# Ajax0564/VyomAI

Measured on AMD Instinct MI355X. Metric: training tokens/sec (12L d=768 seq=512 GPT-style decoder, CLM), higher is better.
Workload: dtype bf16; 1 GPU; configs[1]: GPT-style Decoder 12L d=768 h=12 RoPE vocab 50265, CLM training B=32/GPU seq=512, AdamW, bf16 kernels + fp32 masters; global_batch=32, seq_len=512, parallelism=dp1, attention=none, weights=deterministic recipe (vyomai_amd.recipe)

## Files before the change

include/vyom_hip.h:

```cpp
#ifndef VYOM_HIP_H
#define VYOM_HIP_H

#include <stdint.h>

#ifdef __cplusplus
extern "C" {
#endif

typedef enum { VY_F32 = 0, VY_BF16 = 1 } vy_dtype;

typedef enum {
  VY_OK = 0,
  VY_ERR_ARG = -1,
  VY_ERR_UNSUPPORTED = -2,
  VY_ERR_LAUNCH = -3
} vy_status;

typedef enum {
  VY_ACT_NONE = 0, VY_ACT_GELU_ERF = 1, VY_ACT_GELU_TANH = 2,
  VY_ACT_SILU = 3, VY_ACT_TANH = 4, VY_ACT_SIGMOID = 5, VY_ACT_RELU6 = 6, VY_ACT_LEAKY_RELU = 7
} vy_act;
#define VY_ACT_SAVE_DERIV 0x100

enum {
// ... 11 lines not shown
int vy_workspace_set(void* stream, void* ws, int64_t bytes);

int vy_linear_fwd(const void* x, int64_t ldx, const void* w, int64_t ldw, const void* bias,
                  const void* residual, int64_t ldr, void* y, int64_t ldy, void* pre_out,
                  int64_t M, int64_t N, int64_t K, int act, int dtype, void* stream);

int vy_qkv_rope_fwd(const void* x, int64_t ldx, const void* w, int64_t ldw, const void* bias,
                    const float* cos_tab, const float* sin_tab, int64_t pos0,
                    void* q, int64_t q_sb, int64_t q_sh, int64_t q_sl,
                    void* k, int64_t k_sb, int64_t k_sh, int64_t k_sl,
                    void* v, int64_t v_sb, int64_t v_sh, int64_t v_sl,
                    int64_t B, int64_t L, int64_t K, int h, int hk, int dh, int dtype,
                    void* stream);

int vy_attn_fwd(const void* q, int64_t q_sb, int64_t q_sh, int64_t q_sl,
                const void* k, int64_t k_sb, int64_t k_sh, int64_t k_sl,
                const void* v, int64_t v_sb, int64_t v_sh, int64_t v_sl,
                void* out, int64_t o_sb, int64_t o_sl, float* lse,
                int mask_kind, int64_t start_pos, const uint8_t* keypad, int64_t kp_sb,
                const float* addmask, int64_t am_sb, int64_t am_sl,
                int64_t B, int h, int hk, int64_t L, int64_t S, int dh, float scale, int dtype,
                void* stream);

int vy_attn_decode(const void* q, int64_t q_sb, int64_t q_sh,
                   const void* k, int64_t k_sb, int64_t k_sh, int64_t k_sl,
                   const void* v, int64_t v_sb, int64_t v_sh, int64_t v_sl,
                   void* out, int64_t o_sb, int64_t B, int h, int hk, int64_t S, int dh,
                   float scale, int dtype, void* stream);

int vy_paged_rope_write(void* qkv, int64_t ld, const int32_t* positions, const int64_t* slot_mapping,
                        const float* cos_tab, const float* sin_tab, int64_t table_rows, void* k_cache,
                        void* v_cache, int64_t max_blocks, int block_size, int64_t T, int h, int hk, int dh,
                        int dtype, void* stream);
int vy_attn_paged_decode(const void* q, int64_t q_ld, const int32_t* q_rows, const void* k_cache,
                         const void* v_cache, int64_t max_blocks, int block_size,
                         const int32_t* block_table, int64_t bt_stride, const int32_t* seqlens,
                         int64_t max_seqlen, void* out, int64_t o_ld, int64_t B, int h, int hk, int dh,
                         float scale, int n_split, void* ws, int64_t ws_bytes, int dtype, void* stream);
int64_t vy_attn_paged_decode_ws_bytes(int64_t B, int h, int hk, int dh, int64_t max_seqlen, int n_split, int dtype);
int vy_paged_gather(const void* k_cache, const void* v_cache, int64_t max_blocks, int block_size,
                    const int32_t* block_table, int64_t n_blocks, int64_t S, void* k_out, void* v_out,
                    int hk, int dh, int dtype, void* stream);

int vy_layernorm_fwd(const void* x, int64_t ldx, const void* gamma, const void* beta, void* y,
                     int64_t ldy, float* mean, float* rstd, int64_t M, int64_t N, float eps,
                     int dtype, void* stream);

int vy_rmsnorm_fwd(const void* x, int64_t ldx, const void* w, void* y, int64_t ldy, int64_t M,
                   int64_t N, float eps, float w_offset, int dtype, void* stream);

int vy_gated_act_fwd(const void* gate_up, int64_t ldg, void* out, int64_t ldo, int64_t M, int64_t I,
                     int act, int dtype, void* stream);

int vy_rmsnorm_bwd(const void* dy, int64_t lddy, const void* x, int64_t ldx, const void* w,
                   const void* add_to, int64_t ldadd, void* dx, int64_t lddx, float* dw, float beta,
                   float* ws, int64_t M, int64_t N, float eps, float w_offset, int dtype, void* stream);

int vy_gated_act_bwd(const void* d_act, int64_t lddo, const void* gate_up, int64_t ldg, void* d_gate_up,
                     int64_t lddg, int64_t M, int64_t I, int act, int dtype, void* stream);

int vy_rope_fwd(void* x, int64_t sb, int64_t sh, int64_t sl, const float* cos_tab,
                const float* sin_tab, int64_t pos0, int64_t B, int heads, int64_t L, int dh,
                int inverse, int dtype, void* stream);


int vy_linear_dgrad(const void* dy, int64_t lddy, const void* wt, int64_t ldwt, const void* pre,
                    int64_t ldpre, int act, const void* add_to, int64_t ldadd, const void* add_to2,
                    int64_t ldadd2, void* dx, int64_t lddx, int64_t M, int64_t N, int64_t K, int dtype,
                    void* stream);

int vy_linear_wgrad(const void* dy, int64_t lddy, const void* x, int64_t ldx, float* dw,
                    int64_t lddw, float* db, float beta, const float* alpha_dev, int64_t M, int64_t N,
                    int64_t K, int dtype, void* stream);

typedef struct vy_wgrad_desc {
  const void* dy; int64_t lddy;
  const void* x; int64_t ldx;
  float* dw; int64_t lddw;
  float* db;
  int64_t M, N, K;
} vy_wgrad_desc;
int vy_linear_wgrad_grouped(const vy_wgrad_desc* descs, int32_t n, int dtype, void* stream);

int64_t vy_layernorm_bwd_ws_rows(int64_t M);
int vy_layernorm_bwd(const void* dy, int64_t lddy, const void* x, int64_t ldx, const void* gamma,
                     const float* mean, const float* rstd, void* dx, int64_t lddx, float* dgamma,
                     float* dbeta, float beta, float* ws, int64_t M, int64_t N, int dtype,
                     void* stream);

int vy_attn_bwd(const void* q, int64_t q_sb, int64_t q_sh, int64_t q_sl,
                const void* k, int64_t k_sb, int64_t k_sh, int64_t k_sl,
                const void* v, int64_t v_sb, int64_t v_sh, int64_t v_sl,
                const void* out, const void* dout, int64_t o_sb, int64_t o_sl, const float* lse,
                float* delta_ws,
                void* dq, int64_t dq_sb, int64_t dq_sh, int64_t dq_sl,
                void* dk, int64_t dk_sb, int64_t dk_sh, int64_t dk_sl,
                void* dv, int64_t dv_sb, int64_t dv_sh, int64_t dv_sl,
                int mask_kind, int64_t start_pos, const uint8_t* keypad, int64_t kp_sb,
                const float* cos_tab, const float* sin_tab, int64_t rope_pos0,
                int64_t B, int h, int hk, int64_t L, int64_t S, int dh, float scale, int dtype,
                void* stream);

int vy_ddp_unique_id(void* id128);
int vy_ddp_init(const void* id128, int rank, int world);
int vy_ddp_world(void);
int vy_ddp_rank(void);
int vy_ddp_all_reduce_async(void* buf, int64_t count, int dtype, void* stream);
int vy_ddp_destroy(void);

int vy_adamw_step(float* p, const float* g, float* m, float* v, void* p_bf16, int64_t n, float lr,
                  float beta1, float beta2, float eps, float weight_decay, int64_t step,
                  float grad_scale, const float* grad_scale_dev, void* stream);
int vy_adamw_step_gated(float* p, const float* g, float* m, float* v, void* p_bf16, int64_t n, float lr,
                        float beta1, float beta2, float eps, float weight_decay, int64_t step,
                        float grad_scale, const float* grad_scale_dev, const float* gate, void* stream);

int vy_sumsq(const float* x, int64_t n, float* out, float* ws, void* stream);

int vy_linear_dropout_fwd(const void* x, int64_t ldx, const void* w, int64_t ldw, const void* bias,
                          const void* residual, int64_t ldr, void* y, int64_t ldy, int64_t M, int64_t N,
                          int64_t K, float p_drop, uint64_t seed, uint64_t offset, int dtype, void* stream);
int vy_dropout(const void* x, int64_t ldx, void* y, int64_t ldy, int64_t M, int64_t N, float p_drop,
               uint64_t seed, uint64_t offset, int dtype, void* stream);

int vy_act_bwd(const void* dy, int64_t lddy, const void* pre, int64_t ldpre, void* dx, int64_t lddx,
               int64_t M, int64_t N, int act, int dtype, void* stream);

int vy_xent_fwd(const void* logits, int64_t ld, const int64_t* labels, int64_t ignore_index, float* lse,
                float* loss_sum, float* count, int64_t M, int64_t V, int32_t* err_flag, int dtype, void* stream);
int vy_xent_bwd(void* logits, int64_t ld, const int64_t* labels, int64_t ignore_index, const float* lse,
                const float* gscale, const float* count, int64_t M, int64_t V, int dtype, void* stream);
int vy_xent_fused(void* logits, int64_t ld, const int64_t* labels, int64_t ignore_index, float* lse,
                  float* loss_sum, const float* count, const float* gscale, int64_t M, int64_t V,
                  int32_t* err_flag, int dtype, void* stream);
int vy_xent_sample_fwd(const void* logits, int64_t ld, const int64_t* labels, int64_t ignore_index, float* lse,
                       float* loss_sum, float* count, int64_t* sampled, float inv_temperature, uint64_t seed,
                       uint64_t offset, int64_t M, int64_t V, int32_t* err_flag, int dtype, void* stream);
int vy_xent_sample_fused(void* logits, int64_t ld, const int64_t* labels, int64_t ignore_index, float* lse,
                         float* loss_sum, const float* count, const float* gscale, int64_t* sampled,
                         float inv_temperature, uint64_t seed, uint64_t offset, int64_t M, int64_t V,
                         int32_t* err_flag, int dtype, void* stream);
int vy_gumbel_noise(float* out, int64_t ld, int64_t M, int64_t V, uint64_t seed, uint64_t offset, void* stream);

int vy_bce_head_fwd(const void* h, int64_t ldh, const void* w, const void* b, float* z, const float* target,
                    const uint8_t* live, float* loss_sum, int64_t M, int64_t d, int dtype, void* stream);
int vy_bce_head_bwd(const void* h, int64_t ldh, const void* w, const float* z, const float* target,
                    const uint8_t* live, const float* gscale, const float* count, void* dh, int64_t lddh, float* dw,
                    float* db, int accumulate, int64_t M, int64_t d, int dtype, void* stream);

int vy_mlm_mask(const int64_t* ids, int64_t n, const int64_t* special_ids, int32_t n_special, float fraction,
                int64_t mask_id, int64_t vocab, int64_t ignore_index, uint64_t seed, uint64_t offset,
                int64_t* masked_ids, int64_t* labels, uint8_t* masked, void* stream);


int vy_logprob_fwd(const void* logits, int64_t ld, const int64_t* labels, const float* weight, float* lse,
                   float* logp, int64_t M, int64_t V, int32_t* err_flag, int dtype, void* stream);
int vy_logprob_bwd(void* logits, int64_t ld, const int64_t* labels, const float* weight, const float* lse,
                   int64_t M, int64_t V, int dtype, void* stream);
int vy_logprob_fused(void* logits, int64_t ld, const int64_t* labels, const float* weight, float* lse,
                     float* logp, int64_t M, int64_t V, int32_t* err_flag, int dtype, void* stream);

int vy_embedding_fwd(const void* table, int64_t ldt, const int64_t* ids, void* out, int64_t ldo,
                     int64_t M, int64_t d, int64_t V, int32_t* err_flag, int dtype, void* stream);
int vy_embedding_bwd(const void* dout, int64_t lddo, const int64_t* ids, float* dw, int64_t lddw,
                     int64_t padding_idx, int64_t M, int64_t d, int64_t V, int dtype, void* stream);

int vy_transpose(const void* in, int64_t ldin, void* out, int64_t ldout, int64_t R, int64_t C,
                 int dtype, void* stream);

typedef struct vy_transpose_desc {
  const void* in; void* out;
// ... 64 lines not shown
```

vyomai_amd/_lib.py:

```python
from __future__ import annotations

import ctypes as C
import os
from typing import Optional

_HERE = os.path.dirname(os.path.abspath(__file__))
LIB_PATH = os.environ.get("VY_LIB_PATH") or os.path.join(_HERE, "lib", "libvyom_hip.so")

VY_F32, VY_BF16 = 0, 1
ACT_NONE, ACT_GELU_ERF, ACT_GELU_TANH = 0, 1, 2
ACT_SILU, ACT_TANH, ACT_SIGMOID, ACT_RELU6, ACT_LEAKY_RELU = 3, 4, 5, 6, 7
ACT_SAVE_DERIV = 0x100
MASK_NONE, MASK_CAUSAL, MASK_KEYPAD, MASK_ADDITIVE = 0, 1, 2, 4

_p, _i64, _i, _f, _u64 = C.c_void_p, C.c_int64, C.c_int, C.c_float, C.c_uint64

PROTOTYPES = {
    "vy_linear_fwd": [_p, _i64, _p, _i64, _p, _p, _i64, _p, _i64, _p, _i64, _i64, _i64, _i, _i, _p],
    "vy_qkv_rope_fwd": [_p, _i64, _p, _i64, _p, _p, _p, _i64,
                        _p, _i64, _i64, _i64, _p, _i64, _i64, _i64, _p, _i64, _i64, _i64,
                        _i64, _i64, _i64, _i, _i, _i, _i, _p],
    "vy_attn_fwd": [_p, _i64, _i64, _i64, _p, _i64, _i64, _i64, _p, _i64, _i64, _i64,
                    _p, _i64, _i64, _p, _i, _i64, _p, _i64, _p, _i64, _i64,
                    _i64, _i, _i, _i64, _i64, _i, _f, _i, _p],
    "vy_attn_decode": [_p, _i64, _i64, _p, _i64, _i64, _i64, _p, _i64, _i64, _i64,
                       _p, _i64, _i64, _i, _i, _i64, _i, _f, _i, _p],
    "vy_paged_rope_write": [_p, _i64, _p, _p, _p, _p, _i64, _p, _p, _i64, _i, _i64, _i, _i, _i, _i, _p],
    "vy_attn_paged_decode": [_p, _i64, _p, _p, _p, _i64, _i, _p, _i64, _p, _i64, _p, _i64, _i64, _i, _i, _i, _f, _i,
                             _p, _i64, _i, _p],
    "vy_paged_gather": [_p, _p, _i64, _i, _p, _i64, _i64, _p, _p, _i, _i, _i, _p],
    "vy_layernorm_fwd": [_p, _i64, _p, _p, _p, _i64, _p, _p, _i64, _i64, _f, _i, _p],
    "vy_rmsnorm_fwd": [_p, _i64, _p, _p, _i64, _i64, _i64, _f, _f, _i, _p],
    "vy_gated_act_fwd": [_p, _i64, _p, _i64, _i64, _i64, _i, _i, _p],
    "vy_rmsnorm_bwd": [_p, _i64, _p, _i64, _p, _p, _i64, _p, _i64, _p, _f, _p, _i64, _i64, _f, _f, _i, _p],
    "vy_gated_act_bwd": [_p, _i64, _p, _i64, _p, _i64, _i64, _i64, _i, _i, _p],
    "vy_rope_fwd": [_p, _i64, _i64, _i64, _p, _p, _i64, _i64, _i, _i64, _i, _i, _i, _p],
    "vy_linear_dgrad": [_p, _i64, _p, _i64, _p, _i64, _i, _p, _i64, _p, _i64, _p, _i64, _i64, _i64, _i64, _i, _p],
    "vy_linear_wgrad": [_p, _i64, _p, _i64, _p, _i64, _p, _f, _p, _i64, _i64, _i64, _i, _p],
    "vy_linear_wgrad_grouped": [_p, _i, _i, _p],
    "vy_layernorm_bwd": [_p, _i64, _p, _i64, _p, _p, _p, _p, _i64, _p, _p, _f, _p, _i64, _i64, _i, _p],
    "vy_attn_bwd": [_p, _i64, _i64, _i64, _p, _i64, _i64, _i64, _p, _i64, _i64, _i64,
                    _p, _p, _i64, _i64, _p, _p,
                    _p, _i64, _i64, _i64, _p, _i64, _i64, _i64, _p, _i64, _i64, _i64,
                    _i, _i64, _p, _i64, _p, _p, _i64, _i64, _i, _i, _i64, _i64, _i, _f, _i, _p],
    "vy_adamw_step": [_p, _p, _p, _p, _p, _i64, _f, _f, _f, _f, _f, _i64, _f, _p, _p],
    "vy_adamw_step_gated": [_p, _p, _p, _p, _p, _i64, _f, _f, _f, _f, _f, _i64, _f, _p, _p, _p],
    "vy_sumsq": [_p, _i64, _p, _p, _p],
    "vy_linear_dropout_fwd": [_p, _i64, _p, _i64, _p, _p, _i64, _p, _i64, _i64, _i64, _i64, _f, _u64, _u64, _i, _p],
    "vy_dropout": [_p, _i64, _p, _i64, _i64, _i64, _f, _u64, _u64, _i, _p],
    "vy_act_bwd": [_p, _i64, _p, _i64, _p, _i64, _i64, _i64, _i, _i, _p],
    "vy_xent_fwd": [_p, _i64, _p, _i64, _p, _p, _p, _i64, _i64, _p, _i, _p],
    "vy_xent_bwd": [_p, _i64, _p, _i64, _p, _p, _p, _i64, _i64, _i, _p],
    "vy_xent_fused": [_p, _i64, _p, _i64, _p, _p, _p, _p, _i64, _i64, _p, _i, _p],
    "vy_xent_sample_fwd": [_p, _i64, _p, _i64, _p, _p, _p, _p, _f, _u64, _u64, _i64, _i64, _p, _i, _p],
    "vy_xent_sample_fused": [_p, _i64, _p, _i64, _p, _p, _p, _p, _p, _f, _u64, _u64, _i64, _i64, _p, _i, _p],
    "vy_gumbel_noise": [_p, _i64, _i64, _i64, _u64, _u64, _p],
    "vy_bce_head_fwd": [_p, _i64, _p, _p, _p, _p, _p, _p, _i64, _i64, _i, _p],
    "vy_bce_head_bwd": [_p, _i64, _p, _p, _p, _p, _p, _p, _p, _i64, _p, _p, _i, _i64, _i64, _i, _p],
    "vy_mlm_mask": [_p, _i64, _p, _i, _f, _i64, _i64, _i64, _u64, _u64, _p, _p, _p, _p],
    "vy_logprob_fwd": [_p, _i64, _p, _p, _p, _p, _i64, _i64, _p, _i, _p],
    "vy_logprob_bwd": [_p, _i64, _p, _p, _p, _i64, _i64, _i, _p],
    "vy_logprob_fused": [_p, _i64, _p, _p, _p, _p, _i64, _i64, _p, _i, _p],
    "vy_transpose_batched": [_p, _i, _i, _i, _p],
    "vy_embedding_fwd": [_p, _i64, _p, _p, _i64, _i64, _i64, _i64, _p, _i, _p],
    "vy_embedding_bwd": [_p, _i64, _p, _p, _i64, _i64, _i64, _i64, _i64, _i, _p],
    "vy_transpose": [_p, _i64, _p, _i64, _i64, _i64, _i, _p],
    "vy_greedy_step": [_p, _i64, _i64, _i64, _i, _p, _i64, _i64, _p, _i64, _p, _i, _p, _p, _p],
    "vy_sampling_probs": [_p, _i64, _i64, _i64, _i, _f, _i, _f, _p, _i64, _p],
    "vy_decoder_step": [_p, _p, _i64, _p, _p, _p, _i64, _p],
    "vy_gemma_decoder_step": [_p, _p, _i64, _p, _i64, _p],
    "vy_cast": [_p, _p, _i64, _i, _i, _p],
    "vy_ddp_unique_id": [_p],
    "vy_ddp_init": [_p, _i, _i],
    "vy_ddp_all_reduce_async": [_p, _i64, _i, _p],
    "vy_ddp_destroy": [],
    "vy_set_concurrent_chains": [_i],
    "vy_workspace_set": [_p, _p, _i64],
}
OTHER_SYMBOLS = ["vy_last_error", "vy_abi_version", "vy_layernorm_bwd_ws_rows", "vy_decode_ws_bytes",
                 "vy_gemma_ws_bytes", "vy_ddp_world", "vy_ddp_rank", "vy_attn_paged_decode_ws_bytes"]
ALL_SYMBOLS = list(PROTOTYPES) + OTHER_SYMBOLS


class VyWgradDesc(C.Structure):
    _fields_ = [("dy", _p), ("lddy", _i64), ("x", _p), ("ldx", _i64), ("dw", _p), ("lddw", _i64), ("db", _p),
                ("M", _i64), ("N", _i64), ("K", _i64)]


class VyomHipError(RuntimeError):
    pass


_lib: Optional[C.CDLL] = None


def load() -> C.CDLL:
    global _lib
    if _lib is not None:
        return _lib
    if not os.path.exists(LIB_PATH):
        raise VyomHipError(
            f"{LIB_PATH} is missing: build it with `python -c 'import __graft_entry__ as g; g.build()'` "
            "(hipcc --offload-arch=gfx950).  vyomai_amd has no CPU or PyTorch fallback."
        )
    lib = C.CDLL(LIB_PATH)
    for name, argtypes in PROTOTYPES.items():
        fn = getattr(lib, name)
        fn.argtypes = argtypes
        fn.restype = C.c_int
    lib.vy_last_error.restype = C.c_char_p
    lib.vy_last_error.argtypes = []
    lib.vy_abi_version.restype = C.c_int
    lib.vy_layernorm_bwd_ws_rows.restype = C.c_int64
    lib.vy_layernorm_bwd_ws_rows.argtypes = [_i64]
    lib.vy_decode_ws_bytes.restype = C.c_int64
    lib.vy_decode_ws_bytes.argtypes = [C.c_int32] * 7
    lib.vy_attn_paged_decode_ws_bytes.restype = C.c_int64
    lib.vy_attn_paged_decode_ws_bytes.argtypes = [_i64, _i, _i, _i, _i64, _i, _i]
    _lib = lib
    return lib


def call(name: str, *args) -> None:
    lib = load()
    rc = getattr(lib, name)(*args)
    if rc != 0:
        raise VyomHipError(f"{name} failed ({rc}): {lib.vy_last_error().decode()}")


def dtype_code(torch_dtype) -> int:
    import torch

    if torch_dtype == torch.bfloat16:
        return VY_BF16
    if torch_dtype == torch.float32:
        return VY_F32
    raise VyomHipError(f"vyomai_amd kernels support float32 and bfloat16, got {torch_dtype}")
```

vyomai_amd/autograd_train.py:

```python
from __future__ import annotations

import os

import weakref
from typing import Optional

import torch

from . import _lib, ops
from ._lib import ACT_GELU_ERF, ACT_NONE, VyomHipError
from .layers.attention import _shadow
from .layers.mask import AttnMask
from .layers.positional_embeddings import resolve_freqs

BF16 = torch.bfloat16


WEIGHT_EPOCH = [0]


class _WtRegistry:

    def __init__(self) -> None:
        self.entries = []
# ... 2 lines not shown

    def register(self, owner, key_fn, src_fn, dst):
        e = [weakref.ref(owner), key_fn, src_fn, dst, WEIGHT_EPOCH[0]]
        self.entries.append(e)
        return e

    def refresh(self) -> None:
        ep = WEIGHT_EPOCH[0]
        if self.epoch_done == ep:
            return
        self.epoch_done = ep
        self.entries = [e for e in self.entries if e[0]() is not None]
        live = [e for e in self.entries if e[4] >= ep - 1 and getattr(e[0](), "_vy_wt_key", None) != e[1](e[0]())]
        if not live:
            return
        pairs = [(e[2](e[0]()), e[3]) for e in live]
        for dt in sorted({s_.dtype for s_, _ in pairs}, key=str):
            sub = [(s_, d_) for s_, d_ in pairs if s_.dtype == dt]
            keys = [(s_.data_ptr(), d_.data_ptr()) for s_, d_ in sub]
            batch = self.batches.get(dt)
            if batch is None or batch.keys != keys:
                batch = self.batches[dt] = ops.TransposeBatch(sub)
            batch.run()
        for e in live:
            e[0]()._vy_wt_key = e[1](e[0]())


_WT = _WtRegistry()


def _wt_cached(owner, key_fn, src_fn) -> torch.Tensor:
    view = getattr(owner, "_vy_wt_view", None)
    key = key_fn(owner)
    entry = getattr(owner, "_vy_wt_entry", None)
    if entry is not None:
        entry[4] = WEIGHT_EPOCH[0]
    if view is not None and getattr(owner, "_vy_wt_key", None) == key:
        return view
    src = src_fn(owner)
    if view is not None and view.dtype == src.dtype and view.device == src.device:
        _WT.refresh()
        if owner._vy_wt_key != key:
            ops.transpose(src, view)
            owner._vy_wt_key = key
        return view
    N, K = src.shape
    ld = _row_stride(N)
    view = torch.zeros((K, ld), dtype=src.dtype, device=src.device)[:, :N]
    ops.transpose(src, view)
    owner._vy_wt_view, owner._vy_wt_key = view, key
    owner._vy_wt_entry = _WT.register(owner, key_fn, src_fn, view)
    return view


_ROW_GRANULE = int(os.environ.get("VY_ROW_GRANULE", "64"))


def _row_stride(n: int) -> int:
    g = _ROW_GRANULE
    return (n + g - 1) // g * g


def _wt(param: torch.Tensor, dtype) -> torch.Tensor:
    return _wt_cached(param, lambda p: (p._version, WEIGHT_EPOCH[0], dtype), lambda p: _shadow(p, dtype))


def _direct(p: Optional[torch.Tensor]) -> bool:
    return p is not None and getattr(p, "_vy_direct", False) and p.grad is not None


def _notify(*params) -> None:
    for p in params:
        if p is not None:
            cb = getattr(p, "_vy_ready", None)
            if cb is not None:
                cb(p)


class _WgradGroup:

    TILES = int(os.environ.get("VY_WGRAD_GROUP_TILES", "100"))

    def __init__(self):
        self.items, self.tiles, self.armed = [], 0, False

    def wants(self, dy, w, alpha) -> bool:
        if alpha is not None or not _GROUP_WGRADS:
            return False
        N, K = w.shape
        return dy.numel() // N >= _GROUP_MIN_ROWS and N < 8192 and N * K >= 512 * 512 and K % 8 == 0

    def add(self, dy, x, w, b) -> None:
        self.add_tensors(dy, x, w.grad, None if b is None else b.grad, [p for p in (w, b) if p is not None])

    def add_tensors(self, dy, x, dw, db, members) -> None:
        self.items.append((dy, x, dw, db, members))
        for p in members:
            p._vy_deferred = True
        self.tiles += -(-dw.shape[0] // 256) * -(-dw.shape[1] // 256)
        if not self.armed:
            torch.autograd.Variable._execution_engine.queue_callback(self._end_of_backward)
            self.armed = True
        if self.tiles >= self.TILES or len(self.items) == 8:
            self.flush()

    def flush(self) -> None:
        items, self.items, self.tiles = self.items, [], 0
        if not items:
            return
        ops.linear_wgrad_grouped([(dy, x, dw, db) for dy, x, dw, db, _ in items])
        for *_, members in items:
            for p in members:
                p._vy_deferred = False
            _notify(*members)

    def _end_of_backward(self) -> None:
        self.armed = False
        self.flush()

    def discard(self) -> None:
        for *_, members in self.items:
            for p in members:
                p._vy_deferred = False
        self.items, self.tiles, self.armed = [], 0, False


_GROUP_WGRADS = os.environ.get("VY_WGRAD_GROUP", "1") != "0"
_DEFER_RESIDUALS = os.environ.get("VY_DEFER_RESIDUALS", "1") != "0"
_GROUP_MIN_ROWS = int(os.environ.get("VY_WGRAD_GROUP_ROWS", "2048"))
_GROUP_QKV = os.environ.get("VY_WGRAD_GROUP_QKV", "1") != "0"
_wgrad_group = _WgradGroup()


def _wgrad(dy, x, w: torch.Tensor, b: Optional[torch.Tensor], alpha: Optional[torch.Tensor] = None):
    if _direct(w) and (b is None or _direct(b)):
        if _wgrad_group.wants(dy, w, alpha):
            _wgrad_group.add(dy, x, w, b)
            return None, None
        ops.linear_wgrad(dy, x, w.grad, None if b is None else b.grad, accumulate=True, alpha=alpha)
        _notify(w, b)
        return None, None
    dw = torch.empty(w.shape, dtype=torch.float32, device=w.device)
    db = torch.empty(b.shape, dtype=torch.float32, device=w.device) if b is not None else None
    ops.linear_wgrad(dy, x, dw, db, accumulate=False, alpha=alpha)
    return dw.to(w.dtype), (db.to(b.dtype) if b is not None else None)


def _ln_bwd(dy, x, ln_w, ln_b, mean, rstd):
    dt = x.dtype
    if _direct(ln_w) and _direct(ln_b):
        dx = ops.layernorm_bwd(dy, x, _shadow(ln_w, dt), mean, rstd, ln_w.grad, ln_b.grad, accumulate=True)
        _notify(ln_w, ln_b)
        return dx, None, None
    dg = torch.empty(ln_w.shape, dtype=torch.float32, device=x.device)
    db = torch.empty(ln_b.shape, dtype=torch.float32, device=x.device)
    dx = ops.layernorm_bwd(dy, x, _shadow(ln_w, dt), mean, rstd, dg, db, accumulate=False)
    return dx, dg.to(ln_w.dtype), db.to(ln_b.dtype)


def _defer_list(t: torch.Tensor):
    return getattr(t, "_vy_defer", None) if t is not None else None


def defer_residual_grads(x: torch.Tensor) -> None:
    if torch.is_grad_enabled() and x.requires_grad and _DEFER_RESIDUALS:
        x._vy_defer = []


def _require_bf16(x: torch.Tensor) -> None:
    if x.dtype != BF16 and x.dtype != torch.float32:
        raise VyomHipError("training kernels take bf16 or fp32 activations (fp32 master weights), not %s" % x.dtype)


_EMB_USES = {}
_EMB_WAITING = {}


def reset_embedding_uses() -> None:
    _EMB_USES.clear()
    _EMB_WAITING.clear()


def _embedding_end_of_backward() -> None:
    waiting = list(_EMB_WAITING.values())
    _EMB_WAITING.clear()
    for w in waiting:
        _EMB_USES.pop(id(w), None)
        _notify(w)


class EmbeddingFn(torch.autograd.Function):

    @staticmethod
    def forward(ctx, ids, weight, padding_idx, dtype):
        ctx.save_for_backward(ids)
        ctx.weight, ctx.padding_idx = weight, padding_idx
        if _direct(weight):
            _EMB_USES.setdefault(id(weight), [0, 0])[0] += 1
        return ops.embedding(_shadow(weight, dtype), ids)

    @staticmethod
    def backward(ctx, dout):
        (ids,) = ctx.saved_tensors
        w = ctx.weight
        if _direct(w):
            ops.embedding_bwd_(dout.contiguous(), ids, w.grad, ctx.padding_idx)
            uses = _EMB_USES.get(id(w))
            if uses is not None:
                uses[1] += 1
                if uses[1] < uses[0]:
                    _EMB_WAITING[id(w)] = w
                    torch.autograd.Variable._execution_engine.queue_callback(_embedding_end_of_backward)
                    return None, None, None, None
                del _EMB_USES[id(w)]
                _EMB_WAITING.pop(id(w), None)
            _notify(w)
            return None, None, None, None
        dw = torch.zeros(w.shape, dtype=torch.float32, device=w.device)
        ops.embedding_bwd_(dout.contiguous(), ids, dw, ctx.padding_idx)
        return None, dw.to(w.dtype), None, None


class PatchifyFn(torch.autograd.Function):

    @staticmethod
    def forward(ctx, patches, w, b):
        _require_bf16(patches)
        dt = patches.dtype
        ctx.save_for_backward(patches)
        ctx.params = (w, b)
        return ops.linear(patches, _shadow(w, dt).reshape(w.shape[0], -1), _shadow(b, dt))

    @staticmethod
# ... 756 lines not shown
```

vyomai_amd/csrc/vy_bwd.hip:

```cpp
#include "vy_attn_tile.h"
#include <float.h>
#include <stdlib.h>

namespace {


__device__ __forceinline__ int xcd_remap(int bid, int nwg) {
  const int xcd = bid & 7, q = nwg >> 3, r = nwg & 7;
  return (xcd < r ? xcd * (q + 1) : r * (q + 1) + (xcd - r) * q) + (bid >> 3);
}

__device__ __forceinline__ bf16x8 tr_pair(const char* base, int row_bytes) {
  const s16x4 lo = __builtin_amdgcn_ds_read_tr16_b64_v4i16((VY_LDS s16x4*)(base));
  const s16x4 hi = __builtin_amdgcn_ds_read_tr16_b64_v4i16((VY_LDS s16x4*)(base + 8 * row_bytes));
  union { struct { s16x4 a, b; } s; bf16x8 v; } u;
  u.s.a = lo; u.s.b = hi;
  return u.v;
}

typedef __attribute__((ext_vector_type(2))) __bf16 bf16x2_t;

template <int BT, int MS_, bool MF16>
struct WgradTile {
  static constexpr int MS = MS_;
  static constexpr int NW = BT / 32;
  static constexpr int WKT = BT / 2;
  static constexpr int ROWB = BT * 2;
  static constexpr int TILE = MS * ROWB, STAGE = 2 * TILE;
  static constexpr int PP = TILE / 1024 / NW;
  static_assert(PP * 1024 * NW == TILE, "tile / wave layout mismatch");

  int wave, nst, m_begin, m_end;
  bool ragged;
  int row[PP];
  const bf16* a_ptr[PP]; const bf16* b_ptr[PP];
  int64_t a_step[PP], b_step[PP];
  const bf16* zero;

  __device__ __forceinline__ WgradTile(const bf16* __restrict__ dY, int64_t lddy, const bf16* __restrict__ X, int64_t ldx,
                                       int n0, int k0, int N, int K, int m_begin_, int m_end_, int wave_, int lane) {
    wave = wave_, m_begin = m_begin_, m_end = m_end_;
    nst = (m_end - m_begin + MS - 1) / MS;
    ragged = ((m_end - m_begin) % MS) != 0;
    zero = reinterpret_cast<const bf16*>(vy_zero16);
    sources(dY, lddy, n0, N, lane, a_ptr, a_step);
    sources(X, ldx, k0, K, lane, b_ptr, b_step);
  }
  __device__ __forceinline__ void sources(const bf16* __restrict__ src, int64_t ld, int c0, int C, int lane,
                                          const bf16* (&ptr)[PP], int64_t (&step)[PP]) {
#pragma unroll
    for (int t = 0; t < PP; ++t) {
      const int P = (wave * PP + t) * 1024 + lane * 16;
      const int r = P / ROWB, off = P % ROWB;
      const int col = (off ^ (((r & 3) << 6) | (MF16 ? ((r >> 2) & 1) << 5 : 0))) >> 1;
      const bool ok = c0 + col < C;
      row[t] = r;
      ptr[t] = ok ? src + (int64_t)(m_begin + r) * ld + c0 + col : zero;
      step[t] = ok ? (int64_t)MS * ld : 0;
    }
  }
  __device__ __forceinline__ void issue(const bf16* (&ptr)[PP], const int64_t (&step)[PP], int s, char* dst) {
    const bool tail = ragged && s == nst - 1;
    const int rows = m_end - (m_begin + s * MS);
#pragma unroll
    for (int t = 0; t < PP; ++t) {
      const bf16* p = (tail && row[t] >= rows) ? zero : ptr[t];
      __builtin_amdgcn_global_load_lds((const VY_GLOBAL void*)p, (VY_LDS void*)(dst + (wave * PP + t) * 1024), 16, 0, 0);
      ptr[t] += step[t];
    }
  }
  __device__ __forceinline__ void stage(int s, char* dst) {
    issue(a_ptr, a_step, s, dst);
    issue(b_ptr, b_step, s, dst + TILE);
  }
};

__device__ __forceinline__ float wgrad_db_dot(const bf16x8& a, float s) {
  const bf16x2_t ones2 = {(__bf16)1.0f, (__bf16)1.0f};
  union { bf16x8 v; bf16x2_t h[4]; } u_;
  u_.v = a;
#pragma unroll
  for (int e = 0; e < 4; ++e) s = __builtin_amdgcn_fdot2_f32_bf16(u_.h[e], ones2, s, false);
  return s;
}

// ... 170 lines not shown
    const bool hi = kq >= 2;
#pragma unroll
    for (int i = 0; i < TI; ++i)
#pragma unroll
      for (int jp = 0; jp < JH; ++jp) {
        const int k = kw + 16 * (2 * jp + (hi ? 1 : 0)) + r16;
#pragma unroll
        for (int r = 0; r < 4; ++r) {
          const unsigned x = __builtin_bit_cast(unsigned, acc[i][2 * jp][r] * alpha);
          const unsigned y = __builtin_bit_cast(unsigned, acc[i][2 * jp + 1][r] * alpha);
          auto sw = __builtin_amdgcn_permlane32_swap(x, y, false, false);
          const int nlo = nw + 16 * i + 4 * (kq & 1) + r;
          if (k < K) {
            if (nlo < N) atomicAdd(dW + (int64_t)nlo * lddw + k, __builtin_bit_cast(float, (unsigned)sw[0]));
            if (nlo + 8 < N) atomicAdd(dW + (int64_t)(nlo + 8) * lddw + k, __builtin_bit_cast(float, (unsigned)sw[1]));
          }
        }
      }
  }
};

template <int BN, int BKW, int MS, int NS, bool MF16>
__device__ __forceinline__ void wgrad_tn_bf16_body(
    const bf16* __restrict__ dY, int64_t lddy, const bf16* __restrict__ X, int64_t ldx,
    float* __restrict__ dW, int64_t lddw, float* __restrict__ db, const float* __restrict__ alpha_dev,
    int M, int N, int K, int tiles_k, int tiles_nk, int m_chunk, int diag, int wg) {
  static_assert(BN == BKW && ((BN == 128 && MS == 64 && NS == 2) || (BN == 256 && MS == 32 && NS == 4)),
                "built shapes: 128 x 128 x 64 in 2 stages, 256 x 256 x 32 in 4");
  typedef WgradTile<BN, MS, MF16> Tile;
  typedef std::conditional_t<MF16, WgradMma16<Tile>, WgradMma32<Tile>> Mma;
  constexpr int STAGE = Tile::STAGE, PS = 2 * Tile::PP;
  __shared__ __attribute__((aligned(16))) char smem[NS * STAGE];
  const int tid = threadIdx.x, lane = tid & 63;
  const int wave = __builtin_amdgcn_readfirstlane(tid >> 6);
  const int wn = wave >> 1, wk = wave & 1;
  const int split = wg / tiles_nk, t2 = wg - split * tiles_nk;
  const int tile_n = t2 / tiles_k, tile_k = t2 - tile_n * tiles_k;
  const int n0 = tile_n * BN, k0 = tile_k * BKW;
  const int m_begin = split * m_chunk;
  const int m_end = min(M, m_begin + m_chunk);
  if (m_begin >= m_end) return;

  Tile t(dY, lddy, X, ldx, n0, k0, N, K, m_begin, m_end, wave, lane);
  const bool do_db = db != nullptr && tile_k == 0 && wk == 0;
  Mma mma(smem, lane, wn, wk);
  const int nst = t.nst;
#pragma unroll
  for (int s_ = 0; s_ < NS - 1; ++s_)
    if (s_ < nst) t.stage(s_, smem + s_ * STAGE);
  for (int s = 0; s < nst; ++s) {
    const int younger = min(NS - 2, nst - 1 - s);
    if (younger >= 2) asm volatile("s_waitcnt vmcnt(%0)" ::"n"(2 * PS) : "memory");
    else if (younger == 1) asm volatile("s_waitcnt vmcnt(%0)" ::"n"(PS) : "memory");
    else asm volatile("s_waitcnt vmcnt(0)" ::: "memory");
    __builtin_amdgcn_s_barrier();
    asm volatile("" ::: "memory");
    if (s + NS - 1 < nst) t.stage(s + NS - 1, smem + (s + NS - 1) % NS * STAGE);
    mma.mma_stage(s % NS * STAGE, do_db);
  }
  if (diag == 1) {
    if (mma.acc[0][0][0] == 12345.678f) dW[0] = 1.f;
    return;
  }
  const float alpha = alpha_dev ? *alpha_dev : 1.0f;
  mma.epilogue(dW, lddw, db, do_db, alpha, n0 + wn * 64, k0 + wk * Tile::WKT, N, K);
}

template <int BN, int BKW, int MS, int NS, bool MF16>
__global__ __launch_bounds__(BN * 2, BN == 128 ? 2 : 1) void wgrad_tn_bf16_kernel(
    const bf16* __restrict__ dY, int64_t lddy, const bf16* __restrict__ X, int64_t ldx,
    float* __restrict__ dW, int64_t lddw, float* __restrict__ db, const float* __restrict__ alpha_dev,
    int M, int N, int K, int tiles_k, int tiles_nk, int m_chunk, int diag) {
  wgrad_tn_bf16_body<BN, BKW, MS, NS, MF16>(dY, lddy, X, ldx, dW, lddw, db, alpha_dev, M, N, K, tiles_k, tiles_nk, m_chunk,
                                            diag, xcd_remap(blockIdx.x, gridDim.x));
}

struct WgradItem {
  const bf16* dY; const bf16* X; float* dW; float* db;
  int64_t lddy, ldx, lddw;
  int M, N, K, tiles_k, tiles_nk, m_chunk, item0;
};
struct WgradGroup { WgradItem g[8]; int n; };

template <int BN, int BKW, int MS, int NS, bool MF16>
__global__ __launch_bounds__(BN * 2, 1) void wgrad_tn_bf16_grouped_kernel(WgradGroup grp, int diag) {
  const int id = xcd_remap(blockIdx.x, gridDim.x);
  int d = 0;
#pragma unroll
  for (int i = 1; i < 8; ++i)
    if (i < grp.n && id >= grp.g[i].item0) d = i;
  WgradItem it = grp.g[0];
#pragma unroll
  for (int i = 1; i < 8; ++i)
    if (d == i) it = grp.g[i];
  wgrad_tn_bf16_body<BN, BKW, MS, NS, MF16>(it.dY, it.lddy, it.X, it.ldx, it.dW, it.lddw, it.db, nullptr, it.M, it.N, it.K,
                                            it.tiles_k, it.tiles_nk, it.m_chunk, diag, id - it.item0);
}

__global__ __launch_bounds__(64) void colsum_bf16_kernel(const bf16* __restrict__ dY, int64_t lddy,
                                                         float* __restrict__ db, int M, int N) {
  const int c0 = (blockIdx.x * 64 + threadIdx.x) * 8;
  if (c0 >= N) return;
  const int m0 = blockIdx.y * 256, m1 = min(M, m0 + 256);
  float s[8] = {0, 0, 0, 0, 0, 0, 0, 0};
  for (int m = m0; m < m1; ++m) {
    const bf16x8 v = *reinterpret_cast<const bf16x8*>(dY + (int64_t)m * lddy + c0);
#pragma unroll
    for (int e = 0; e < 8; ++e) s[e] += (float)v[e];
  }
#pragma unroll
  for (int e = 0; e < 8; ++e)
    if (c0 + e < N) atomicAdd(db + c0 + e, s[e]);
}

struct BwdParams {
  const bf16* q; int64_t q_sb, q_sh, q_sl;
  const bf16* k; int64_t k_sb, k_sh, k_sl;
  const bf16* v; int64_t v_sb, v_sh, v_sl;
  const bf16* o; const bf16* dout; int64_t o_sb, o_sl;
  const float* lse; float* delta;
  bf16* dq; int64_t dq_sb, dq_sh, dq_sl;
  bf16* dk; int64_t dk_sb, dk_sh, dk_sl;
  bf16* dv; int64_t dv_sb, dv_sh, dv_sl;
  int mask_kind; int start_pos;
  const uint8_t* keypad; int64_t kp_sb;
  int B, h, hk, L, S;
  float scale;
  const float* cos_tab; const float* sin_tab; int rope_pos0;
};

__global__ __launch_bounds__(256, 3) void attn_bwd_dq_kernel(BwdParams p) {
  constexpr int DH = 64, RB = 128, NS = 3, KPW = 256;
  typedef AttnStage<RB, NS> Stage;
  constexpr int TILE = Stage::TILE;
  __shared__ __attribute__((aligned(16))) char smem[2 * NS * TILE + KPW * 8];
  const AttnLane ln;
  const AttnQBlock blk(p, ln);
  const int wave = ln.wave, fr = ln.fr, fh = ln.fh;
  const int head = blk.head, b = blk.b, q0 = blk.q0, qi = blk.qi, qrow = blk.qrow;
  const bf16 *Q = blk.Q, *Kb = blk.Kb, *Vb = blk.Vb;
  const bf16* dO = p.dout + (int64_t)b * p.o_sb + (int64_t)qrow * p.o_sl + head * DH;
  bf16x8 qf[4], gf[4];
#pragma unroll
  for (int ks = 0; ks < 4; ++ks) {
    qf[ks] = *reinterpret_cast<const bf16x8*>(Q + ks * 16 + fh * 8);
    gf[ks] = *reinterpret_cast<const bf16x8*>(dO + ks * 16 + fh * 8);
  }
  const int64_t stat = ((int64_t)b * p.h + head) * p.L + qrow;
  const float c = p.scale * LOG2E;
  float neg_lse = -p.lse[stat] * LOG2E;
  float neg_delta;
  {
    const bf16* Op = p.o + (int64_t)b * p.o_sb + (int64_t)qrow * p.o_sl + head * DH;
    float acc_ = 0.f;
#pragma unroll
    for (int ks = 0; ks < 4; ++ks) {
      const bf16x8 of = *reinterpret_cast<const bf16x8*>(Op + ks * 16 + fh * 8);
#pragma unroll
      for (int e = 0; e < 8; ++e) acc_ += (float)of[e] * (float)gf[ks][e];
    }
    acc_ += __shfl_xor(acc_, 32, 64);
    neg_delta = -acc_;
    if (fh == 0 && qi < p.L) p.delta[stat] = neg_delta;
  }
  const bool causal = p.mask_kind & VY_MASK_CAUSAL;
  const bool haskp = p.mask_kind & VY_MASK_KEYPAD;
  const uint8_t* kp = haskp ? p.keypad + (int64_t)b * p.kp_sb : nullptr;

  const Stage st_w(ln, SwDual{}, SwRows<RB>{});
// ... 292 lines not shown
    sb[lr][lc] = colsum;
    __syncthreads();
    if (tid < 64 && n0 + tid < N) atomicAdd(db + n0 + tid, alpha * (sb[0][tid] + sb[1][tid] + sb[2][tid] + sb[3][tid]));
  }
}

int wgrad_f32(const char* who, const void* dy, int64_t lddy, const void* x, int64_t ldx, float* dw, int64_t lddw, float* db,
              float beta, const float* alpha_dev, int64_t M, int64_t N, int64_t K, hipStream_t st) {
  if (beta == 0.f) {
    if (hipMemset2DAsync(dw, lddw * sizeof(float), 0, K * sizeof(float), N, st) != hipSuccess)
      VY_FAIL(VY_ERR_LAUNCH, "%s: memset failed", who);
    if (db && hipMemsetAsync(db, 0, N * sizeof(float), st) != hipSuccess) VY_FAIL(VY_ERR_LAUNCH, "%s: memset failed", who);
  }
  const int tiles_k = (int)vy_cdiv(K, 64), tiles = (int)vy_cdiv(N, 64) * tiles_k;
  int64_t splits = vy_cdiv(1024, tiles);
  const int64_t max_splits = vy_cdiv(M, 64);
  if (splits > max_splits) splits = max_splits;
  if (splits < 1) splits = 1;
  const int64_t m_chunk = vy_cdiv(vy_cdiv(M, splits), 16) * 16;
  splits = vy_cdiv(M, m_chunk);
  hipLaunchKernelGGL(wgrad_tn_f32_kernel, dim3((unsigned)(tiles * splits)), dim3(256), 0, st, (const float*)dy, lddy,
                     (const float*)x, ldx, dw, lddw, db, alpha_dev, (int)M, (int)N, (int)K, tiles_k, tiles, (int)m_chunk);
  VY_CHECK_LAUNCH(who);
  return VY_OK;
}

bool wgrad_bf16_operands_ok(const void* dy, int64_t lddy, const void* x, int64_t ldx, int64_t N, int64_t K) {
  return !(K % 8 || lddy % 8 || ldx % 8 || lddy < vy_cdiv(N, 8) * 8 || (uintptr_t)dy % 16 || (uintptr_t)x % 16);
}

struct WgradSplit { int64_t splits, m_chunk; };
WgradSplit wgrad_split(int64_t M, int64_t want) {
  const int64_t max_splits = vy_cdiv(M, 256);
  if (want > max_splits) want = max_splits;
  if (want < 1) want = 1;
  const int64_t m_chunk = vy_cdiv(vy_cdiv(M, want), 64) * 64;
  return {vy_cdiv(M, m_chunk), m_chunk};
}

int wgrad_env(const char* name, int dflt) { const char* e = getenv(name); return e ? atoi(e) : dflt; }

int wgrad_m16() { static const int v = wgrad_env("VY_WGRAD_M16", 1); return v; }
int wgrad_diag() { static const int v = wgrad_env("VY_WGRAD_DIAG", 0); return v; }

}

extern "C" int vy_linear_wgrad(const void* dy, int64_t lddy, const void* x, int64_t ldx, float* dw,
                               int64_t lddw, float* db, float beta, const float* alpha_dev, int64_t M,
                               int64_t N, int64_t K, int dtype, void* stream) {
  const char* who = "vy_linear_wgrad";
  if (dtype != VY_BF16 && dtype != VY_F32) VY_FAIL(VY_ERR_ARG, "%s: bad dtype %d", who, dtype);
  if (!dy || !x || !dw || M <= 0 || N <= 0 || K <= 0) VY_FAIL(VY_ERR_ARG, "%s: bad arguments", who);
  if (dtype == VY_F32) {
    if (beta != 0.f && beta != 1.f) VY_FAIL(VY_ERR_ARG, "%s: beta must be 0 or 1", who);
    return wgrad_f32(who, dy, lddy, x, ldx, dw, lddw, db, beta, alpha_dev, M, N, K, (hipStream_t)stream);
  }
  if (!wgrad_bf16_operands_ok(dy, lddy, x, ldx, N, K))
    VY_FAIL(VY_ERR_ARG, "%s: K and leading dimensions must be multiples of 8 (lddy >= roundup8(N)), operands 16-byte aligned", who);
  if (beta != 0.f && beta != 1.f) VY_FAIL(VY_ERR_ARG, "%s: beta must be 0 or 1", who);
  static const int wv = wgrad_env("VY_WGRAD_VARIANT", -1);
  static const int tgt = wgrad_env("VY_WGRAD_TARGET", 0);
  if (wv != -1 && wv != 0 && wv != 8)
    VY_FAIL(VY_ERR_UNSUPPORTED, "%s: VY_WGRAD_VARIANT=%d was removed (the values left are 0 and 8; unset selects by shape)", who, wv);
  hipStream_t st = (hipStream_t)stream;
  if (beta == 0.f) {
    if (hipMemset2DAsync(dw, lddw * sizeof(float), 0, K * sizeof(float), N, st) != hipSuccess)
      VY_FAIL(VY_ERR_LAUNCH, "%s: memset failed", who);
    if (db && hipMemsetAsync(db, 0, N * sizeof(float), st) != hipSuccess)
      VY_FAIL(VY_ERR_LAUNCH, "%s: memset failed", who);
  }
  const bool big = wv < 0 ? (N >= 8192 && M >= 4096) : wv == 8;
  const int BT = big ? 256 : 128;
  const int tiles_k = (int)vy_cdiv(K, BT), tiles = (int)vy_cdiv(N, BT) * tiles_k;
  const WgradSplit sp = wgrad_split(M, tgt > 0 ? vy_cdiv(tgt, tiles) : big ? 256 / tiles : vy_cdiv(384, tiles));
  const int w16 = wgrad_m16();
  auto kernel = big ? (w16 ? wgrad_tn_bf16_kernel<256, 256, 32, 4, true> : wgrad_tn_bf16_kernel<256, 256, 32, 4, false>)
                    : (w16 >= 2 ? wgrad_tn_bf16_kernel<128, 128, 64, 2, true> : wgrad_tn_bf16_kernel<128, 128, 64, 2, false>);
  hipLaunchKernelGGL(kernel, dim3((unsigned)(tiles * sp.splits)), dim3(BT * 2), 0, st, (const bf16*)dy, lddy, (const bf16*)x,
                     ldx, dw, lddw, db, alpha_dev, (int)M, (int)N, (int)K, tiles_k, tiles, (int)sp.m_chunk, wgrad_diag());
  VY_CHECK_LAUNCH(who);
  return VY_OK;
}

extern "C" int vy_linear_wgrad_grouped(const vy_wgrad_desc* descs, int32_t n, int dtype, void* stream) {
  const char* who = "vy_linear_wgrad_grouped";
  if (dtype != VY_BF16 && dtype != VY_F32) VY_FAIL(VY_ERR_ARG, "%s: bad dtype %d", who, dtype);
  if (!descs || n <= 0 || n > 8) VY_FAIL(VY_ERR_ARG, "%s: 1..8 descriptors", who);
  if (dtype == VY_F32) {
    for (int i = 0; i < n; ++i) {
      const vy_wgrad_desc& d = descs[i];
      if (!d.dy || !d.x || !d.dw || d.M <= 0 || d.N <= 0 || d.K <= 0) VY_FAIL(VY_ERR_ARG, "%s: descriptor %d: bad arguments", who, i);
      if (int rc = wgrad_f32(who, d.dy, d.lddy, d.x, d.ldx, d.dw, d.lddw, d.db, 1.f, nullptr, d.M, d.N, d.K, (hipStream_t)stream)) return rc;
    }
    return VY_OK;
  }
  int64_t tiles_total = 0;
  for (int i = 0; i < n; ++i) {
    const vy_wgrad_desc& d = descs[i];
    if (!d.dy || !d.x || !d.dw || d.M <= 0 || d.N <= 0 || d.K <= 0) VY_FAIL(VY_ERR_ARG, "%s: descriptor %d: bad arguments", who, i);
    if (!wgrad_bf16_operands_ok(d.dy, d.lddy, d.x, d.ldx, d.N, d.K))
      VY_FAIL(VY_ERR_ARG, "%s: descriptor %d: K and leading dimensions must be multiples of 8, operands 16-byte aligned", who, i);
    tiles_total += vy_cdiv(d.N, 256) * vy_cdiv(d.K, 256);
  }
  static const int tgt = wgrad_env("VY_WGRAD_GROUP_TARGET", 256);
  WgradGroup grp;
  grp.n = n;
  int64_t items = 0;
  for (int i = 0; i < n; ++i) {
    const vy_wgrad_desc& d = descs[i];
    const int64_t tiles_k = vy_cdiv(d.K, 256), tiles = vy_cdiv(d.N, 256) * tiles_k;
    const WgradSplit sp = wgrad_split(d.M, tgt / tiles_total);
    WgradItem& it = grp.g[i];
    it.dY = (const bf16*)d.dy; it.X = (const bf16*)d.x; it.dW = d.dw; it.db = d.db;
    it.lddy = d.lddy; it.ldx = d.ldx; it.lddw = d.lddw;
    it.M = (int)d.M; it.N = (int)d.N; it.K = (int)d.K;
    it.tiles_k = (int)tiles_k; it.tiles_nk = (int)tiles; it.m_chunk = (int)sp.m_chunk; it.item0 = (int)items;
    items += tiles * sp.splits;
  }
  for (int i = n; i < 8; ++i) grp.g[i] = grp.g[0];
  auto kernel = wgrad_m16() ? wgrad_tn_bf16_grouped_kernel<256, 256, 32, 4, true> : wgrad_tn_bf16_grouped_kernel<256, 256, 32, 4, false>;
  hipLaunchKernelGGL(kernel, dim3((unsigned)items), dim3(512), 0, (hipStream_t)stream, grp, wgrad_diag());
  VY_CHECK_LAUNCH(who);
  return VY_OK;
}

namespace {

template <int DHP>
struct GenBwd {
  static constexpr int PITCH = (DHP + 8) * 2, KS = DHP / 32, NDB = DHP / 16, CPRW = DHP / 8, CPT = 64 * CPRW / 256;
};

__device__ __forceinline__ float gen_groups_sum(float v) {
  const unsigned u = __builtin_bit_cast(unsigned, v);
  auto s16 = __builtin_amdgcn_permlane16_swap(u, u, false, false);
  v = __builtin_bit_cast(float, (unsigned)s16[0]) + __builtin_bit_cast(float, (unsigned)s16[1]);
  const unsigned w = __builtin_bit_cast(unsigned, v);
  auto s32 = __builtin_amdgcn_permlane32_swap(w, w, false, false);
  return __builtin_bit_cast(float, (unsigned)s32[0]) + __builtin_bit_cast(float, (unsigned)s32[1]);
}

template <int DHP>
__device__ __forceinline__ void gen_stage(char* dst, const bf16* src, int64_t sl, int row0, int nrows, int dh, int tid,
                                          bf16x8 (&reg)[GenBwd<DHP>::CPT]) {
  (void)dst;
  constexpr int CPRW = GenBwd<DHP>::CPRW, CPT = GenBwd<DHP>::CPT;
  const bf16x8 zero8 = {(bf16)0.f, (bf16)0.f, (bf16)0.f, (bf16)0.f, (bf16)0.f, (bf16)0.f, (bf16)0.f, (bf16)0.f};
#pragma unroll
  for (int i = 0; i < CPT; ++i) {
    const int cidx = tid + 256 * i;
    const int row = cidx / CPRW, ch = cidx - row * CPRW;
    const int r = row0 + row;
    const bool ok = ch * 8 < dh && r < nrows;
    reg[i] = ok ? *reinterpret_cast<const bf16x8*>(src + (int64_t)r * sl + ch * 8) : zero8;
  }
}
template <int DHP>
__device__ __forceinline__ void gen_store(char* dst, int tid, const bf16x8 (&reg)[GenBwd<DHP>::CPT]) {
  constexpr int CPRW = GenBwd<DHP>::CPRW, CPT = GenBwd<DHP>::CPT, PITCH = GenBwd<DHP>::PITCH;
#pragma unroll
  for (int i = 0; i < CPT; ++i) {
    const int cidx = tid + 256 * i;
    const int row = cidx / CPRW, ch = cidx - row * CPRW;
    *reinterpret_cast<bf16x8*>(dst + row * PITCH + ch * 16) = reg[i];
  }
}

template <int DHP>
__global__ __launch_bounds__(256) void attn_bwd_gen_dq_kernel(BwdParams p, int dh) {
  typedef GenBwd<DHP> G;
  constexpr int PITCH = G::PITCH, KS = G::KS, NDB = G::NDB, CPT = G::CPT;
  __shared__ __attribute__((aligned(16))) char smem[2 * 64 * PITCH];
  char* kt = smem;
  char* vt = smem + 64 * PITCH;
  const int tid = threadIdx.x, lane = tid & 63;
  const int wave = __builtin_amdgcn_readfirstlane(tid >> 6);
  const int r16 = lane & 15, kq = lane >> 4;
  const int head = (int)blockIdx.x % p.h, b = (int)blockIdx.x / p.h;
  const int kvh = head / (p.h / p.hk);
  const int q0 = ((int)gridDim.y - 1 - (int)blockIdx.y) * 64;
  const int qi = q0 + wave * 16 + r16;
  const int qrow = qi < p.L ? qi : p.L - 1;
  const bf16* Q = p.q + (int64_t)b * p.q_sb + (int64_t)head * p.q_sh + (int64_t)qrow * p.q_sl;
  const bf16* dO = p.dout + (int64_t)b * p.o_sb + (int64_t)qrow * p.o_sl + head * dh;
  const bf16* Op = p.o + (int64_t)b * p.o_sb + (int64_t)qrow * p.o_sl + head * dh;
  const bf16* Kb = p.k + (int64_t)b * p.k_sb + (int64_t)kvh * p.k_sh;
  const bf16* Vb = p.v + (int64_t)b * p.v_sb + (int64_t)kvh * p.v_sh;
  const bool causal = p.mask_kind & VY_MASK_CAUSAL;
  const bool haskp = p.mask_kind & VY_MASK_KEYPAD;
  const uint8_t* kp = haskp ? p.keypad + (int64_t)b * p.kp_sb : nullptr;
  const bf16x8 zero8 = {(bf16)0.f, (bf16)0.f, (bf16)0.f, (bf16)0.f, (bf16)0.f, (bf16)0.f, (bf16)0.f, (bf16)0.f};
  bf16x8 qf[KS], gf[KS];
  float dacc = 0.f;
#pragma unroll
  for (int ks = 0; ks < KS; ++ks) {
    const int d0 = 32 * ks + 8 * kq;
    qf[ks] = d0 < dh ? *reinterpret_cast<const bf16x8*>(Q + d0) : zero8;
    gf[ks] = d0 < dh ? *reinterpret_cast<const bf16x8*>(dO + d0) : zero8;
    const bf16x8 of = d0 < dh ? *reinterpret_cast<const bf16x8*>(Op + d0) : zero8;
#pragma unroll
    for (int e = 0; e < 8; ++e) dacc += (float)of[e] * (float)gf[ks][e];
  }
  const float neg_delta = -gen_groups_sum(dacc);
  const int64_t stat = ((int64_t)b * p.h + head) * p.L + qrow;
  if (kq == 0 && qi < p.L) p.delta[stat] = neg_delta;
  const float c = p.scale * LOG2E;
// ... 447 lines not shown
```

vyomai_amd/csrc/vy_common.h:

```cpp
#pragma once
#include <hip/hip_runtime.h>
#include <type_traits>
#include <stdint.h>
#include <stdio.h>
#include <math.h>
#include "../../include/vyom_hip.h"

typedef __bf16 bf16;
typedef __attribute__((ext_vector_type(8))) __bf16 bf16x8;
typedef __attribute__((ext_vector_type(4))) __bf16 bf16x4;
typedef __attribute__((ext_vector_type(2))) __bf16 bf16x2;
typedef __attribute__((ext_vector_type(4))) short s16x4;
typedef __attribute__((ext_vector_type(16))) float f32x16;
typedef __attribute__((ext_vector_type(4))) float f32x4;
typedef __attribute__((ext_vector_type(2))) float f32x2;
typedef __attribute__((ext_vector_type(4))) unsigned int u32x4;
typedef __attribute__((ext_vector_type(2))) unsigned int u32x2;

#define VY_LDS __attribute__((address_space(3)))
#define VY_GLOBAL __attribute__((address_space(1)))

__device__ __forceinline__ s16x4 vy_lds_tr16(const char* p) {
  s16x4 r;
  asm volatile("ds_read_b64_tr_b16 %0, %1" : "=v"(r) : "v"((unsigned)(uintptr_t)(VY_LDS const char*)p) : "memory");
  return r;
}
template <int OFF>
__device__ __forceinline__ s16x4 vy_lds_tr16_off(unsigned lds_addr) {
  static_assert(OFF >= 0 && OFF < 65536, "ds offset field is 16 bits");
  s16x4 r;
  asm volatile("ds_read_b64_tr_b16 %0, %1 offset:%2" : "=v"(r) : "v"(lds_addr), "n"(OFF) : "memory");
  return r;
}
template <int OFF0, int OFF1>
__device__ __forceinline__ bf16x8 vy_lds_tr16_pair_off(unsigned lds_addr) {
  union { struct { s16x4 a, b; } s; bf16x8 v; } u;
  u.s.a = vy_lds_tr16_off<OFF0>(lds_addr);
  u.s.b = vy_lds_tr16_off<OFF1>(lds_addr);
  return u.v;
}
template <int OFF>
__device__ __forceinline__ bf16x8 vy_lds_read128_off(unsigned lds_addr) {
  static_assert(OFF >= 0 && OFF < 65536, "ds offset field is 16 bits");
  bf16x8 r;
  asm volatile("ds_read_b128 %0, %1 offset:%2" : "=v"(r) : "v"(lds_addr), "n"(OFF) : "memory");
  return r;
}
__device__ __forceinline__ unsigned vy_lds_addr(const char* p) { return (unsigned)(uintptr_t)(VY_LDS const char*)p; }
__device__ __forceinline__ bf16x8 vy_lds_tr16_pair(const char* p0, const char* p1) {
  union { struct { s16x4 a, b; } s; bf16x8 v; } u;
  u.s.a = vy_lds_tr16(p0);
  u.s.b = vy_lds_tr16(p1);
  return u.v;
}
template <int N, typename F>
__device__ __forceinline__ void vy_static_for(F&& f) {
  if constexpr (N > 0) {
    vy_static_for<N - 1>(f);
    f(std::integral_constant<int, N - 1>{});
  }
}
template <typename T>
__device__ __forceinline__ void vy_tie(T& v) { asm volatile("" : "+v"(v)); }
template <int N, typename... T>
__device__ __forceinline__ void vy_lgkm_wait(T&... v) {
  asm volatile("s_waitcnt lgkmcnt(%0)" ::"n"(N) : "memory");
  (vy_tie(v), ...);
}

void vy_set_error(const char* fmt, ...);
#define VY_FAIL(code, ...)      \
  do {                          \
    vy_set_error(__VA_ARGS__);  \
    return (code);              \
  } while (0)
#define VY_CHECK_LAUNCH(name)                                             \
  do {                                                                    \
    hipError_t e_ = hipGetLastError();                                    \
    if (e_ != hipSuccess)                                                 \
      VY_FAIL(VY_ERR_LAUNCH, "%s: %s", name, hipGetErrorString(e_));      \
  } while (0)

static inline int64_t vy_cdiv(int64_t a, int64_t b) { return (a + b - 1) / b; }

static __device__ __attribute__((aligned(16))) uint32_t vy_zero16[4] = {0, 0, 0, 0};

__device__ __forceinline__ float vy_gelu_erf(float x) {
  return 0.5f * x * (1.0f + erff(x * 0.70710678118654752440f));
}
__device__ __forceinline__ float vy_gelu_erf_grad(float x) {
  const float cdf = 0.5f * (1.0f + erff(x * 0.70710678118654752440f));
  const float pdf = 0.39894228040143267794f * __expf(-0.5f * x * x);
  return cdf + x * pdf;
}
__device__ __forceinline__ float vy_gelu_tanh(float x) {
  const float c = 0.79788456080286535588f;
  return 0.5f * x * (1.0f + tanhf(c * (x + 0.044715f * x * x * x)));
}
__device__ __forceinline__ float vy_gelu_tanh_grad(float x) {
  const float c = 0.79788456080286535588f;
  const float u = c * (x + 0.044715f * x * x * x);
  const float t = tanhf(u);
  return 0.5f * (1.0f + t) + 0.5f * x * (1.0f - t * t) * c * (1.0f + 3.0f * 0.044715f * x * x);
}
__device__ __forceinline__ void vy_phi_fast(float x, float& cdf, float& gauss) {
  const float ax = fabsf(x) * 0.70710678118654752440f;
  const float t = __builtin_amdgcn_rcpf(1.0f + 0.3275911f * ax);
  gauss = __expf(-ax * ax);
  float poly = 1.061405429f;
  poly = poly * t - 1.453152027f;
  poly = poly * t + 1.421413741f;
  poly = poly * t - 0.284496736f;
  poly = poly * t + 0.254829592f;
  const float erf_abs = 1.0f - poly * t * gauss;
  cdf = 0.5f * (1.0f + copysignf(erf_abs, x));
}
__device__ __forceinline__ float vy_gelu_erf_fast(float x) {
  float cdf, g;
  vy_phi_fast(x, cdf, g);
  return x * cdf;
}
__device__ __forceinline__ float vy_gelu_erf_grad_fast(float x) {
  float cdf, g;
  vy_phi_fast(x, cdf, g);
  return cdf + x * 0.39894228040143267794f * g;
}

constexpr float VY_LEAKY_SLOPE = 0.01f;
__device__ __forceinline__ float vy_sigmoid(float x) { return 1.0f / (1.0f + expf(-x)); }
__device__ __forceinline__ float vy_sigmoid_fast(float x) { return __builtin_amdgcn_rcpf(1.0f + __expf(-x)); }
__device__ __forceinline__ float vy_tanh_fast(float x) { return 1.0f - 2.0f * __builtin_amdgcn_rcpf(1.0f + __expf(2.0f * x)); }
__device__ __forceinline__ float vy_relu6(float x) { return fminf(fmaxf(x, 0.0f), 6.0f); }
__device__ __forceinline__ float vy_relu6_grad(float x) { return (x > 0.0f && x < 6.0f) ? 1.0f : 0.0f; }
__device__ __forceinline__ float vy_leaky_relu(float x) { return x > 0.0f ? x : VY_LEAKY_SLOPE * x; }
__device__ __forceinline__ float vy_leaky_relu_grad(float x) { return x > 0.0f ? 1.0f : VY_LEAKY_SLOPE; }

constexpr int VY_ACT_RUNTIME = 0x40;

template <int ACT>
__device__ __forceinline__ float vy_act_fwd(float x) {
  static_assert(ACT != VY_ACT_RUNTIME, "resolve the run-time code with vy_act_dispatch first");
  if constexpr (ACT == VY_ACT_GELU_ERF) return vy_gelu_erf(x);
  else if constexpr (ACT == VY_ACT_GELU_TANH) return vy_gelu_tanh(x);
  else if constexpr (ACT == VY_ACT_SILU) return x * vy_sigmoid(x);
  else if constexpr (ACT == VY_ACT_TANH) return tanhf(x);
  else if constexpr (ACT == VY_ACT_SIGMOID) return vy_sigmoid(x);
  else if constexpr (ACT == VY_ACT_RELU6) return vy_relu6(x);
  else if constexpr (ACT == VY_ACT_LEAKY_RELU) return vy_leaky_relu(x);
  else return x;
}
template <int ACT>
__device__ __forceinline__ float vy_act_grad(float x) {
  static_assert(ACT != VY_ACT_RUNTIME, "resolve the run-time code with vy_act_dispatch first");
  if constexpr (ACT == VY_ACT_GELU_ERF) return vy_gelu_erf_grad(x);
  else if constexpr (ACT == VY_ACT_GELU_TANH) return vy_gelu_tanh_grad(x);
  else if constexpr (ACT == VY_ACT_SILU) { const float s = vy_sigmoid(x); return s * (1.0f + x * (1.0f - s)); }
  else if constexpr (ACT == VY_ACT_TANH) { const float t = tanhf(x); return 1.0f - t * t; }
  else if constexpr (ACT == VY_ACT_SIGMOID) { const float s = vy_sigmoid(x); return s * (1.0f - s); }
  else if constexpr (ACT == VY_ACT_RELU6) return vy_relu6_grad(x);
  else if constexpr (ACT == VY_ACT_LEAKY_RELU) return vy_leaky_relu_grad(x);
  else return 1.0f;
}

template <int ACT, typename F>
__device__ __forceinline__ void vy_act_dispatch(int code, F&& f) {
  if constexpr (ACT != VY_ACT_RUNTIME) {
    f(std::integral_constant<int, ACT>{});
// ... 143 lines not shown
```

vyomai_amd/csrc/vy_gemm.hip:

```cpp
#include "vy_common.h"

int vy_rope_qk(void* q, int64_t q_sb, int64_t q_sh, int64_t q_sl, int hq, void* k, int64_t k_sb, int64_t k_sh,
               int64_t k_sl, int hk, const float* cos_tab, const float* sin_tab, int64_t pos0, int64_t B, int64_t L, int dh,
               int dtype, hipStream_t st);

#include <stdlib.h>
#include <mutex>

namespace {


template <typename T> struct Quad;
template <> struct Quad<bf16> {
  static __device__ __forceinline__ void load(const bf16* p, float (&v)[4]) {
    bf16x4 t = *reinterpret_cast<const bf16x4*>(p);
#pragma unroll
    for (int e = 0; e < 4; ++e) v[e] = (float)t[e];
  }
  static __device__ __forceinline__ void store(bf16* p, const float (&v)[4]) {
    bf16x4 t;
#pragma unroll
    for (int e = 0; e < 4; ++e) t[e] = (bf16)v[e];
    *reinterpret_cast<bf16x4*>(p) = t;
  }
};
template <> struct Quad<float> {
  static __device__ __forceinline__ void load(const float* p, float (&v)[4]) {
    f32x4 t = *reinterpret_cast<const f32x4*>(p);
#pragma unroll
    for (int e = 0; e < 4; ++e) v[e] = t[e];
  }
  static __device__ __forceinline__ void store(float* p, const float (&v)[4]) {
    f32x4 t = {v[0], v[1], v[2], v[3]};
    *reinterpret_cast<f32x4*>(p) = t;
  }
};

template <typename T> __device__ __forceinline__ float round_like(float x);
template <> __device__ __forceinline__ float round_like<bf16>(float x) { return vy_round_bf16(x); }
template <> __device__ __forceinline__ float round_like<float>(float x) { return x; }

template <typename T>
struct EpiPlain {
  const T* bias;
  const T* residual; int64_t ldr;
  const T* residual2; int64_t ldr2;
  const T* gradpre;  int64_t ldg;
  T* y;   int64_t ldy;
  T* pre;
  int vec_ok;
  VyDrop drop;
  int wt_store;
  int pre_deriv;
  int act;
};

template <typename T, int ACT, bool GRAD>
__device__ __forceinline__ void epi_plain_quad_act(const EpiPlain<T>& e, float (&v)[4], int64_t m, int n,
                                                   int N) {
  if (n >= N) return;
  const bool full = e.vec_ok && (n + 3 < N);
  if (full) {
    if (e.bias) { float b[4]; Quad<T>::load(e.bias + n, b);
#pragma unroll
      for (int i = 0; i < 4; ++i) v[i] += b[i]; }
    if (e.pre) {
      if (e.pre_deriv) { float dv[4];
#pragma unroll
        for (int i = 0; i < 4; ++i) dv[i] = vy_act_grad<ACT>(round_like<T>(v[i]));
        Quad<T>::store(e.pre + m * e.ldy + n, dv);
      } else Quad<T>::store(e.pre + m * e.ldy + n, v);
    }
    if constexpr (!GRAD) {
#pragma unroll
      for (int i = 0; i < 4; ++i) v[i] = vy_act_fwd<ACT>(v[i]);
      if (e.drop.thr) {
        uint32_t lots[4];
        vy_drop_lots(e.drop, m, n >> 3, lots);
#pragma unroll
        for (int i = 0; i < 4; ++i) v[i] = vy_drop_keep(e.drop, lots, (n & 7) + i) ? round_like<T>(v[i]) * e.drop.scale : 0.f;
      }
    } else {
      if (e.gradpre) { float g[4]; Quad<T>::load(e.gradpre + m * e.ldg + n, g);
#pragma unroll
        for (int i = 0; i < 4; ++i) v[i] *= e.pre_deriv ? g[i] : vy_act_grad<ACT>(g[i]); }
    }
    if (e.residual) { float r[4]; Quad<T>::load(e.residual + m * e.ldr + n, r);
#pragma unroll
      for (int i = 0; i < 4; ++i) v[i] += r[i]; }
    if (e.residual2) { float r[4]; Quad<T>::load(e.residual2 + m * e.ldr2 + n, r);
#pragma unroll
      for (int i = 0; i < 4; ++i) v[i] += r[i]; }
    Quad<T>::store(e.y + m * e.ldy + n, v);
  } else {
#pragma unroll
    for (int i = 0; i < 4; ++i) {
      if (n + i >= N) break;
      float x = v[i];
      if (e.bias) x += VyT<T>::ld(e.bias + n + i);
      if (e.pre) VyT<T>::st(e.pre + m * e.ldy + n + i, e.pre_deriv ? vy_act_grad<ACT>(round_like<T>(x)) : x);
      if constexpr (!GRAD) {
        x = vy_act_fwd<ACT>(x);
        if (e.drop.thr) {
          uint32_t lots[4];
          vy_drop_lots(e.drop, m, (n + i) >> 3, lots);
          x = vy_drop_keep(e.drop, lots, (n + i) & 7) ? round_like<T>(x) * e.drop.scale : 0.f;
        }
      }
      else if (e.gradpre) { const float gg = VyT<T>::ld(e.gradpre + m * e.ldg + n + i); x *= e.pre_deriv ? gg : vy_act_grad<ACT>(gg); }
      if (e.residual) x += VyT<T>::ld(e.residual + m * e.ldr + n + i);
      if (e.residual2) x += VyT<T>::ld(e.residual2 + m * e.ldr2 + n + i);
      VyT<T>::st(e.y + m * e.ldy + n + i, x);
    }
  }
}

template <typename T, int ACT, bool GRAD>
__device__ __forceinline__ void epi_plain_quad(const EpiPlain<T>& e, float (&v)[4], int64_t m, int n,
                                               int N) {
  if constexpr (ACT != VY_ACT_RUNTIME) epi_plain_quad_act<T, ACT, GRAD>(e, v, m, n, N);
  else vy_act_dispatch<ACT>(e.act, [&](auto a) __attribute__((always_inline)) { epi_plain_quad_act<T, decltype(a)::value, GRAD>(e, v, m, n, N); });
}

template <int ACT>
__device__ __forceinline__ float gradpre_factor_fast(float g, int pre_deriv, int code) {
  if constexpr (ACT != VY_ACT_RUNTIME) {
    return pre_deriv ? g : vy_act_grad_fast<ACT>(g);
  } else {
    float r = g;
    if (!pre_deriv) vy_act_dispatch<ACT>(code, [&](auto a) __attribute__((always_inline)) { r = vy_act_grad_fast<decltype(a)::value>(g); });
    return r;
  }
}

template <int ACT>
__device__ __forceinline__ void epi_chunk_act(const EpiPlain<bf16>& ep, float (&v)[8], bool dual, int64_t m, int n, int N) {
  if (dual && ep.pre_deriv) {
// ... 42 lines not shown
  n -= e.nq;
  if (n < e.nkv) return e.k + b * e.k_sb + (n >> 6) * e.k_sh + lkv * e.k_sl + d;
  n -= e.nkv;
  return e.v + b * e.v_sb + (n >> 6) * e.v_sh + lkv * e.v_sl + d;
}

template <typename T>
__device__ __forceinline__ T* qkv_dest(const EpiQkv<T>& e, int64_t b, int64_t l, int n) {
  if (n < e.nq) { const int hd = n / e.dh, d = n - hd * e.dh;
    return e.q + b * e.q_sb + hd * e.q_sh + l * e.q_sl + d; }
  n -= e.nq;
  if (e.pos_dev) l += *e.pos_dev;
  if (n < e.nkv) { const int hd = n / e.dh, d = n - hd * e.dh;
    return e.k + b * e.k_sb + hd * e.k_sh + l * e.k_sl + d; }
  n -= e.nkv;
  const int hd = n / e.dh, d = n - hd * e.dh;
  return e.v + b * e.v_sb + hd * e.v_sh + l * e.v_sl + d;
}


template <typename T>
__device__ __forceinline__ void epi_qkv_pair(const EpiQkv<T>& e, float (&lo)[4], float (&hi)[4],
                                             int64_t m, int n_lo, int N) {
  if (n_lo >= N) return;
  const int64_t b = m / e.L, l = m - b * e.L;
  if (e.bias) {
    float b0[4], b1[4];
    Quad<T>::load(e.bias + n_lo, b0); Quad<T>::load(e.bias + n_lo + 32, b1);
#pragma unroll
    for (int i = 0; i < 4; ++i) { lo[i] += b0[i]; hi[i] += b1[i]; }
  }
  if (e.rope && n_lo < e.nq + e.nkv) {
    const int d = n_lo & 31;
    const int64_t pp = (e.pos_dev ? (int64_t)*e.pos_dev : e.pos0) + l;
    const float* cp = e.cos_tab + pp * 32 + d;
    const float* sp = e.sin_tab + pp * 32 + d;
    const f32x4 c4 = *reinterpret_cast<const f32x4*>(cp);
    const f32x4 s4 = *reinterpret_cast<const f32x4*>(sp);
#pragma unroll
    for (int i = 0; i < 4; ++i) {
      const float c = round_like<T>(c4[i]), s = round_like<T>(s4[i]);
      const float a = round_like<T>(lo[i]), bb = round_like<T>(hi[i]);
      lo[i] = round_like<T>(a * c) - round_like<T>(bb * s);
      hi[i] = round_like<T>(bb * c) + round_like<T>(a * s);
    }
  }
  Quad<T>::store(qkv_dest(e, b, l, n_lo), lo);
  Quad<T>::store(qkv_dest(e, b, l, n_lo + 32), hi);
}

template <typename T>
__device__ __forceinline__ void epi_qkv_quad(const EpiQkv<T>& e, float (&v)[4], int64_t m, int n, int N) {
  if (n >= N) return;
  const int64_t b = m / e.L, l = m - b * e.L;
  if (e.bias) { float b0[4]; Quad<T>::load(e.bias + n, b0);
#pragma unroll
    for (int i = 0; i < 4; ++i) v[i] += b0[i]; }
  Quad<T>::store(qkv_dest(e, b, l, n), v);
}

__device__ unsigned long long vy_gemm_clk[6];
constexpr int VY_KNOB_ROT = 1;
constexpr int VY_KNOB_CLK = 16;
constexpr int VY_KNOB_NO_BAND = 32;
#define VY_CLK_BEGIN(on)                                                         \
  const bool clk_on_ = (on) && blockIdx.x == 0 && threadIdx.x == 0;              \
  unsigned long long clk_c0_ = 0, clk_w0_ = 0, clk_m_ = 0;                       \
  if (clk_on_) { clk_c0_ = clk_m_ = __builtin_readcyclecounter(); clk_w0_ = wall_clock64(); }
#define VY_CLK_MARK(i)                                                           \
  if (clk_on_) {                                                                 \
    const unsigned long long now_ = __builtin_readcyclecounter();                \
    atomicAdd(&vy_gemm_clk[3 + (i)], now_ - clk_m_);                             \
    clk_m_ = now_;                                                               \
  }
#define VY_CLK_END()                                                             \
  if (clk_on_) {                                                                 \
    atomicAdd(&vy_gemm_clk[0], __builtin_readcyclecounter() - clk_c0_);          \
    atomicAdd(&vy_gemm_clk[1], wall_clock64() - clk_w0_);                        \
    atomicAdd(&vy_gemm_clk[2], 1ull);                                            \
  }

int g_chains = 1;
int g_gemm_variant = -2;
inline bool vy_m16_on() {
  static const int v = [] { const char* e = getenv("VY_GEMM_M16"); return e ? atoi(e) : 1; }();
  return v != 0;
}
inline int vy_gemm_variant() {
  if (g_gemm_variant == -2) { const char* e = getenv("VY_GEMM_VARIANT"); g_gemm_variant = e ? atoi(e) : -1; }
  return g_gemm_variant;
}

__device__ __forceinline__ int xcd_remap(int bid, int nwg) {
  const int xcd = bid & 7, q = nwg >> 3, r = nwg & 7;
  return (xcd < r ? xcd * (q + 1) : r * (q + 1) + (xcd - r) * q) + (bid >> 3);
}

__device__ __forceinline__ void tile_of(int bid, int nwg, int tiles_n, int band_on, int& tile_m, int& tile_n) {
  const int tiles_m = nwg / tiles_n;
  if (band_on && tiles_n >= 8 && (tiles_n & 1) == 0 && (tiles_m & 3) == 0 && tiles_m * tiles_n == nwg) {
    const int xcd = bid & 7, i = bid >> 3;
    const int band = xcd & 1, grp = xcd >> 1;
    const int bw = tiles_n >> 1, pg = tiles_m >> 2;
    tile_m = grp * pg + i / bw;
    tile_n = band * bw + i - (i / bw) * bw;
  } else {
    const int wg = xcd_remap(bid, nwg);
    tile_m = wg / tiles_n;
    tile_n = wg - tile_m * tiles_n;
  }
}

constexpr int BK = 64;
constexpr int ROWB = BK * 2;

constexpr int epi_tile_bytes(int BM, int BN, int PASSES) { return (BM / PASSES) * (BN * 2 + 16); }
constexpr bool epi_has_rope_tab(int BM, int BN, int EPI, int PASSES) {
  return EPI == 1 && epi_tile_bytes(BM, BN, PASSES) + (BM / PASSES) * 128 <= 160 * 1024;
}
constexpr int epi_lds_bytes(int BM, int BN, int EPI, int PASSES) {
  return epi_tile_bytes(BM, BN, PASSES) + (epi_has_rope_tab(BM, BN, EPI, PASSES) ? (BM / PASSES) * 128 : 0);
}
constexpr int vy_cmax(int a, int b) { return a > b ? a : b; }

template <int BM, int BN, int WGM, int WGN, bool MF16> struct AccTile {
  typedef f32x16 T32[BN / (32 * WGN)][BM / (32 * WGM)];
  typedef f32x4 T16[BN / (16 * WGN)][BM / (16 * WGM)];
  typedef std::conditional_t<MF16, T16, T32> type;
};

template <int BM, int BN, int WGM, int WGN, int EPI, int ACT, bool GRAD, int PASSES = 1, bool PF_OK = true, bool MF16 = false>
__device__ __forceinline__ void gemm_epilogue(typename AccTile<BM, BN, WGM, WGN, MF16>::type& acc, char* smem,
                                              int m0, int n0, int M, int N, const EpiPlain<bf16>& ep,
                                              const EpiQkv<bf16>& eq) {
  static_assert(!MF16 || PASSES == 1, "the 16 x 16 accumulator layout is staged in one pass");
  constexpr int NW = WGM * WGN, NT = 64 * NW;
  constexpr int TM = BM / (32 * WGM), TN = BN / (32 * WGN);
  constexpr int EROW = BN * 2 + 16;
  constexpr int RP = BM / PASSES;
  static_assert(WGM % PASSES == 0, "a pass must be whole wave rows");
  const int tid = threadIdx.x, lane = tid & 63;
  const int wave = __builtin_amdgcn_readfirstlane(tid >> 6);
  const int wm = wave / WGN, wn = wave % WGN;
  const int fr = lane & 31, fh = lane >> 5;
  constexpr int CPR = BN / 8;
  char* et = smem;

  const int my_pass = (wm * 32 * TM) / RP;
  auto stage_quad = [&](int row, int col, const float (&v)[4]) {
    bf16x4 w;
#pragma unroll
    for (int e = 0; e < 4; ++e) w[e] = (bf16)v[e];
    *reinterpret_cast<bf16x4*>(et + (row - my_pass * RP) * EROW + col * 2) = w;
  };
  const bf16* biasp = EPI == 0 ? ep.bias : eq.bias;
  const bool bias_vec = (reinterpret_cast<uintptr_t>(biasp) & 7) == 0;
  auto bias_quad = [&](int n, float (&bq)[4]) {
    if (biasp && n + 3 < N && bias_vec) {
      const bf16x4 b4 = *reinterpret_cast<const bf16x4*>(biasp + n);
#pragma unroll
      for (int e = 0; e < 4; ++e) bq[e] = (float)b4[e];
    } else {
#pragma unroll
      for (int e = 0; e < 4; ++e) bq[e] = (biasp && n + e < N) ? (float)biasp[n + e] : 0.f;
    }
  };
  auto stage_all = [&](int pass) {
    if constexpr (!MF16) {
      if (PASSES == 1 || pass == my_pass) {
#pragma unroll
        for (int i = 0; i < TN; ++i)
#pragma unroll
          for (int rg = 0; rg < 4; ++rg) {
            float bq[4];
            bias_quad(n0 + wn * 32 * TN + i * 32 + 8 * rg + 4 * fh, bq);
#pragma unroll
            for (int j = 0; j < TM; ++j) {
              float v[4];
#pragma unroll
              for (int e = 0; e < 4; ++e) v[e] = acc[i][j][4 * rg + e] + bq[e];
              stage_quad(wm * 32 * TM + j * 32 + fr, wn * 32 * TN + i * 32 + 8 * rg + 4 * fh, v);
            }
          }
      }
    } else {
      constexpr int TM16 = BM / (16 * WGM), TN16 = BN / (16 * WGN);
      const int r16 = lane & 15, kq = lane >> 4;
#pragma unroll
      for (int i = 0; i < TN16; ++i) {
        float bq[4];
        bias_quad(n0 + wn * 16 * TN16 + 16 * i + 4 * kq, bq);
#pragma unroll
        for (int j = 0; j < TM16; ++j) {
          float v[4];
#pragma unroll
          for (int e = 0; e < 4; ++e) v[e] = acc[i][j][e] + bq[e];
          stage_quad(wm * 16 * TM16 + 16 * j + r16, wn * 16 * TN16 + 16 * i + 4 * kq, v);
        }
      }
    }
  };

  if constexpr (EPI == 0) {
    const bf16* pf_ptr = GRAD ? (ep.gradpre ? ep.gradpre : ep.residual) : ep.residual;
    const int64_t pf_ld = GRAD ? (ep.gradpre ? ep.ldg : ep.ldr) : ep.ldr;
    const bool pf_is_gradpre = GRAD && ep.gradpre != nullptr;
    auto do_chunk = [&](bf16* __restrict__ dst, bool dual, int pass, int c, bool pf, const bf16x8& p8) {
        const int row = c / CPR, cc = c - row * CPR;
        const int64_t m = m0 + pass * RP + row;
        const int n = n0 + cc * 8;
        if (m >= M || n >= N) return;
        const bf16x8 sv = *reinterpret_cast<const bf16x8*>(et + row * EROW + cc * 16);
        float v[8];
#pragma unroll
        for (int e = 0; e < 8; ++e) v[e] = (float)sv[e];
        if (dual && !ep.pre_deriv) {
          if (ep.vec_ok && n + 8 <= N) {
            *reinterpret_cast<bf16x8*>(ep.pre + m * ep.ldy + n) = sv;
          } else {
            for (int e = 0; e < 8 && n + e < N; ++e) ep.pre[m * ep.ldy + n + e] = sv[e];
          }
        }
        if constexpr (!GRAD && ACT != VY_ACT_NONE) {
          if constexpr (ACT != VY_ACT_RUNTIME) epi_chunk_act<ACT>(ep, v, dual, m, n, N);
          else vy_act_dispatch<ACT>(ep.act, [&](auto a) __attribute__((always_inline)) { epi_chunk_act<decltype(a)::value>(ep, v, dual, m, n, N); });
        }
        if constexpr (!GRAD) {
          if (ep.drop.thr) {
            uint32_t lots[4];
            vy_drop_lots(ep.drop, m, n >> 3, lots);
#pragma unroll
            for (int e = 0; e < 8; ++e) v[e] = vy_drop_keep(ep.drop, lots, e) ? v[e] * ep.drop.scale : 0.f;
          }
        }
        if (ep.vec_ok && n + 8 <= N) {
          if constexpr (GRAD) {
            if (ep.gradpre) {
              const bf16x8 g = pf ? p8 : *reinterpret_cast<const bf16x8*>(ep.gradpre + m * ep.ldg + n);
#pragma unroll
              for (int e = 0; e < 8; ++e) v[e] *= gradpre_factor_fast<ACT>((float)g[e], ep.pre_deriv, ep.act);
            }
          }
          if (ep.residual) {
            const bf16x8 r = (pf && !pf_is_gradpre) ? p8 : *reinterpret_cast<const bf16x8*>(ep.residual + m * ep.ldr + n);
#pragma unroll
            for (int e = 0; e < 8; ++e) v[e] += (float)r[e];
          }
          if (ep.residual2) {
            const bf16x8 r = *reinterpret_cast<const bf16x8*>(ep.residual2 + m * ep.ldr2 + n);
#pragma unroll
            for (int e = 0; e < 8; ++e) v[e] += (float)r[e];
          }
          bf16x8 o;
#pragma unroll
          for (int e = 0; e < 8; ++e) o[e] = (bf16)v[e];
          if (ep.wt_store) {
            asm volatile("global_store_dwordx4 %0, %1, off sc1\n\ts_nop 1" ::"v"(dst + m * ep.ldy + n), "v"(o) : "memory");
          } else {
            *reinterpret_cast<bf16x8*>(dst + m * ep.ldy + n) = o;
          }
        } else {
          for (int e = 0; e < 8 && n + e < N; ++e) {
            float x = v[e];
            if constexpr (GRAD) {
              if (ep.gradpre) { const float gg = (float)ep.gradpre[m * ep.ldg + n + e]; x *= gradpre_factor_fast<ACT>(gg, ep.pre_deriv, ep.act); }
            }
            if (ep.residual) x += (float)ep.residual[m * ep.ldr + n + e];
            if (ep.residual2) x += (float)ep.residual2[m * ep.ldr2 + n + e];
            dst[m * ep.ldy + n + e] = (bf16)x;
          }
        }
    };
    constexpr bool PFK = PF_OK && PASSES == 1 && BM * BN == 256 * 192 && (RP * CPR) % NT == 0;
    constexpr int ITERS = PFK ? (RP * CPR) / NT : 1;
    bf16x8 pre8[ITERS];
    const bool pf_on = PFK && pf_ptr != nullptr && ep.vec_ok && m0 + BM <= M && n0 + BN <= N;
    if constexpr (PFK) {
      if (pf_on) {
#pragma unroll
        for (int it = 0; it < ITERS; ++it) {
          const int c = tid + it * NT;
          const int row = c / CPR, cc = c - row * CPR;
          pre8[it] = *reinterpret_cast<const bf16x8*>(pf_ptr + (int64_t)(m0 + row) * pf_ld + n0 + cc * 8);
        }
      }
    }
    auto flush_plain = [&](bf16* __restrict__ dst, bool final_pass, bool dual, int pass) {
      (void)final_pass;
      if constexpr (PFK) {
        if (pf_on) {
#pragma unroll
          for (int it = 0; it < ITERS; ++it) do_chunk(dst, dual, pass, tid + it * NT, true, pre8[it]);
          return;
        }
      }
      const bf16x8 none{};
      for (int c = tid; c < RP * CPR; c += NT) do_chunk(dst, dual, pass, c, false, none);
    };
    const bool dual = !GRAD && ep.pre != nullptr;
#pragma unroll 1
    for (int pass = 0; pass < PASSES; ++pass) {
      stage_all(pass);
      __syncthreads();
      flush_plain(ep.y, true, dual, pass);
      if (pass + 1 < PASSES) __syncthreads();
    }
  } else {
    constexpr bool TAB = epi_has_rope_tab(BM, BN, 1, PASSES);
    char* rt = smem + RP * EROW;
    const bool use_tab = TAB && eq.rope && n0 < eq.nq + eq.nkv;
    const unsigned Lu = (unsigned)eq.L;
    const unsigned b0 = (unsigned)m0 / Lu, l0 = (unsigned)m0 - b0 * Lu;
    const int64_t pdev = eq.pos_dev ? (int64_t)*eq.pos_dev : 0;
    const int64_t pbase = eq.pos_dev ? pdev : eq.pos0;
#pragma unroll 1
    for (int pass = 0; pass < PASSES; ++pass) {
    constexpr int TIT = (RP * 8 + NT - 1) / NT;
    f32x4 tv[TAB ? TIT : 1][2];
    if constexpr (TAB) {
      if (use_tab) {
#pragma unroll
        for (int it = 0; it < TIT; ++it) {
          const int idx = tid + it * NT;
          const int row = idx >> 3, ch = idx & 7;
          if (RP * 8 % NT == 0 || idx < RP * 8) {
            const unsigned t = l0 + (unsigned)(pass * RP + row);
            const unsigned l = t - (t / Lu) * Lu;
            const float* src = (ch < 4 ? eq.cos_tab : eq.sin_tab) + (pbase + l) * 32 + (ch & 3) * 8;
            tv[it][0] = *reinterpret_cast<const f32x4*>(src);
            tv[it][1] = *reinterpret_cast<const f32x4*>(src + 4);
          }
        }
      }
    }
    stage_all(pass);
    if constexpr (TAB) {
      if (use_tab) {
#pragma unroll
        for (int it = 0; it < TIT; ++it) {
          const int idx = tid + it * NT;
          if (RP * 8 % NT == 0 || idx < RP * 8) {
            bf16x8 o;
#pragma unroll
            for (int e = 0; e < 4; ++e) { o[e] = (bf16)tv[it][0][e]; o[4 + e] = (bf16)tv[it][1][e]; }
            *reinterpret_cast<bf16x8*>(rt + idx * 16) = o;
          }
        }
      }
    }
    __syncthreads();
    for (int c = tid; c < RP * CPR; c += NT) {
      const int row = c / CPR, cc = c - row * CPR;
      const int64_t m = m0 + pass * RP + row;
      const int n = n0 + cc * 8;
      if (m >= M || n >= N) continue;
      const unsigned t = l0 + (unsigned)(pass * RP + row);
      const unsigned tq = t / Lu;
      const int64_t b = b0 + tq, l = t - tq * Lu;
      bf16x8 sv = *reinterpret_cast<const bf16x8*>(et + row * EROW + cc * 16);
      if (eq.rope && n < eq.nq + eq.nkv) {
        const bf16x8 pv = *reinterpret_cast<const bf16x8*>(et + row * EROW + (cc ^ 4) * 16);
        const int d = n & 31;
        const bool hi = (n & 32) != 0;
        float cs[8], sn[8];
        if (TAB && use_tab) {
          const bf16x8 c8 = *reinterpret_cast<const bf16x8*>(rt + row * 128 + (d >> 3) * 16);
          const bf16x8 s8 = *reinterpret_cast<const bf16x8*>(rt + row * 128 + 64 + (d >> 3) * 16);
#pragma unroll
          for (int e = 0; e < 8; ++e) { cs[e] = (float)c8[e]; sn[e] = (float)s8[e]; }
        } else {
          const float* cp = eq.cos_tab + (pbase + l) * 32 + d;
          const float* sp = eq.sin_tab + (pbase + l) * 32 + d;
#pragma unroll
          for (int e = 0; e < 8; ++e) { cs[e] = vy_round_bf16(cp[e]); sn[e] = vy_round_bf16(sp[e]); }
        }
#pragma unroll
        for (int e = 0; e < 8; ++e) {
          const float a = (float)sv[e], o = (float)pv[e];
          const float t1 = vy_round_bf16(a * cs[e]);
          const float t2 = vy_round_bf16((hi ? o : -o) * sn[e]);
          sv[e] = (bf16)(t1 + t2);
        }
      }
      if (eq.vec8 && eq.dh == 64) {
        *reinterpret_cast<bf16x8*>(qkv_dest64(eq, b, l, n, l + pdev)) = sv;
// ... 1091 lines not shown
    const int tn = (int)vy_cdiv(N, 128), tm = (int)vy_cdiv(M, 32);
    hipLaunchKernelGGL((gemm_nt_bf16_kernel<32, 128, 1, 4, EPI, ACT, GRAD>), dim3(tm * tn), dim3(256), 0,
                       st, X, ldx, W, ldw, (int)M, (int)N, (int)K, tn, ep, eq, rot);
  } else if (M <= 1024 || (mid_tiles && vy_cdiv(M, 256) * vy_cdiv(N, 192) * g_chains < 160)) {
    const int tn = (int)vy_cdiv(N, 128), tm = (int)vy_cdiv(M, 128);
    static const int mid16 = [] { const char* e = getenv("VY_GEMM_MID16"); return e ? atoi(e) : 1; }();
    static const int rows_on = [] { const char* e = getenv("VY_GEMM_ROWS"); return e ? atoi(e) : 1; }();
    if (mid16 && rows_on && M > 128 && M <= 320) {
      if (M <= 256) launch_mid<256, 128, 4, 2, EPI, ACT, GRAD>(X, ldx, W, ldw, M, N, K, ep, eq, st, 256, rot);
      else launch_mid<320, 128, 4, 2, EPI, ACT, GRAD>(X, ldx, W, ldw, M, N, K, ep, eq, st, 256, rot);
    } else if (mid16)
      launch_mid<128, 128, 2, 2, EPI, ACT, GRAD>(X, ldx, W, ldw, M, N, K, ep, eq, st, 448, rot);
    else
      hipLaunchKernelGGL((gemm_nt_bf16_kernel<128, 128, 2, 2, EPI, ACT, GRAD>), dim3(tm * tn), dim3(256), 0,
                         st, X, ldx, W, ldw, (int)M, (int)N, (int)K, tn, ep, eq, rot);
  } else {
    const int tn = (int)vy_cdiv(N, 192), tm = (int)vy_cdiv(M, 256);
    const int tn2 = (int)vy_cdiv(N, 256);
    switch (large_m_kernel(vy_gemm_variant(), vy_m16_on(), N >= 3072)) {
      case LargeM::K32_256x256:
        hipLaunchKernelGGL((gemm_nt_bf16_kernel<256, 256, 4, 2, EPI, ACT, GRAD>), dim3(tm * tn2), dim3(512), 0,
                           st, X, ldx, W, ldw, (int)M, (int)N, (int)K, tn2, ep, eq, rot);
        break;
      case LargeM::K32_256x192:
        hipLaunchKernelGGL((gemm_nt_bf16_kernel<256, 192, 4, 2, EPI, ACT, GRAD>), dim3(tm * tn), dim3(512), 0,
                           st, X, ldx, W, ldw, (int)M, (int)N, (int)K, tn, ep, eq, rot);
        break;
      case LargeM::M16_256x256:
        hipLaunchKernelGGL((gemm_nt_bf16_m16_kernel<256, 256, 4, 2, EPI, ACT, GRAD>), dim3(tm * tn2), dim3(512), 0,
                           st, X, ldx, W, ldw, (int)M, (int)N, (int)K, tn2, ep, eq, rot);
        break;
      case LargeM::X3M16_256x192:
        hipLaunchKernelGGL((gemm_nt_bf16_x3m16_kernel<192, EPI, ACT, GRAD>), dim3(tm * tn), dim3(512), 0,
                           st, X, ldx, W, ldw, (int)M, (int)N, (int)K, tn, ep, eq, rot);
        break;
    }
  }
  return 0;
}

template <int EPI, int ACT, bool GRAD>
int launch_f32(const float* X, int64_t ldx, const float* W, int64_t ldw, int64_t M, int64_t N,
               int64_t K, const EpiPlain<float>& ep, const EpiQkv<float>& eq, hipStream_t st) {
  const int tn = (int)vy_cdiv(N, 64), tm = (int)vy_cdiv(M, 64);
  hipLaunchKernelGGL((gemm_nt_f32_kernel<EPI, ACT, GRAD>), dim3(tm * tn), dim3(256), 0, st, X, ldx, W,
                     ldw, (int)M, (int)N, (int)K, tn, ep, eq);
  return 0;
}

inline bool aligned_to(const void* p, size_t a) { return (reinterpret_cast<uintptr_t>(p) % a) == 0; }

template <typename T>
int check_operands(const char* who, const void* x, int64_t ldx, const void* w, int64_t ldw, int64_t M,
                   int64_t N, int64_t K) {
  const int vec = 16 / (int)sizeof(T);
  if (!x || !w) VY_FAIL(VY_ERR_ARG, "%s: null operand", who);
  if (M <= 0 || N <= 0 || K <= 0) VY_FAIL(VY_ERR_ARG, "%s: empty problem M=%ld N=%ld K=%ld", who, (long)M, (long)N, (long)K);
  if (M > INT32_MAX || N > INT32_MAX || K > INT32_MAX) VY_FAIL(VY_ERR_ARG, "%s: dimension overflow", who);
  if (K % vec) VY_FAIL(VY_ERR_ARG, "%s: K=%ld must be a multiple of %d", who, (long)K, vec);
  if (ldx % vec || ldw % vec || !aligned_to(x, 16) || !aligned_to(w, 16))
    VY_FAIL(VY_ERR_ARG, "%s: operand rows must be 16-byte aligned (ldx=%ld ldw=%ld)", who, (long)ldx, (long)ldw);
  if (ldx < K || ldw < K) VY_FAIL(VY_ERR_ARG, "%s: leading dimension smaller than K", who);
  return 0;
}

template <typename T>
int linear_impl(const void* x, int64_t ldx, const void* w, int64_t ldw, const void* bias,
                const void* residual, int64_t ldr, const void* gradpre, int64_t ldg, void* y,
                int64_t ldy, void* pre_out, int64_t M, int64_t N, int64_t K, int act, bool grad,
                hipStream_t st, const char* who, const void* residual2 = nullptr, int64_t ldr2 = 0,
                VyDrop drop = VyDrop{}) {
  if (int rc = check_operands<T>(who, x, ldx, w, ldw, M, N, K)) return rc;
  if (!y) VY_FAIL(VY_ERR_ARG, "%s: null output", who);
  if (ldy < N) VY_FAIL(VY_ERR_ARG, "%s: ldy < N", who);
  EpiPlain<T> ep;
  ep.pre_deriv = (act & VY_ACT_SAVE_DERIV) ? 1 : 0;
  act &= ~VY_ACT_SAVE_DERIV;
  ep.act = act;
  ep.bias = (const T*)bias; ep.residual = (const T*)residual; ep.ldr = ldr;
  ep.residual2 = (const T*)residual2; ep.ldr2 = ldr2;
  if (residual2 && !residual) VY_FAIL(VY_ERR_ARG, "%s: add_to2 without add_to", who);
  ep.gradpre = (const T*)gradpre; ep.ldg = ldg; ep.y = (T*)y; ep.ldy = ldy; ep.pre = (T*)pre_out;
  ep.drop = drop;
  static const int wt_env = [] { const char* e = getenv("VY_GEMM_WT_STORE"); return e ? atoi(e) : 1; }();
  ep.wt_store = (wt_env && (int64_t)M * N * (int64_t)sizeof(T) >= (16 << 20)) ? 1 : 0;
  const int ve = 16 / (int)sizeof(T);
  ep.vec_ok = (ldy % ve == 0) && aligned_to(y, 16) && (!bias || aligned_to(bias, 4 * sizeof(T))) &&
              (!residual || (ldr % ve == 0 && aligned_to(residual, 16))) &&
              (!residual2 || (ldr2 % ve == 0 && aligned_to(residual2, 16))) &&
              (!gradpre || (ldg % ve == 0 && aligned_to(gradpre, 16))) &&
              (!pre_out || aligned_to(pre_out, 16));
  EpiQkv<T> eq{};
#define VY_GO(ACT_, GRAD_)                                                                              \
  do {                                                                                                  \
    if constexpr (sizeof(T) == 2)                                                                       \
      launch_bf16<0, ACT_, GRAD_>((const bf16*)x, ldx, (const bf16*)w, ldw, M, N, K,                    \
                                  *reinterpret_cast<EpiPlain<bf16>*>(&ep), *reinterpret_cast<EpiQkv<bf16>*>(&eq), st); \
    else                                                                                                \
      launch_f32<0, ACT_, GRAD_>((const float*)x, ldx, (const float*)w, ldw, M, N, K,                   \
                                 *reinterpret_cast<EpiPlain<float>*>(&ep), *reinterpret_cast<EpiQkv<float>*>(&eq), st); \
  } while (0)
  if (!grad) {
    if (act == VY_ACT_NONE) VY_GO(VY_ACT_NONE, false);
    else if (act == VY_ACT_GELU_ERF) VY_GO(VY_ACT_GELU_ERF, false);
    else if (act == VY_ACT_GELU_TANH) VY_GO(VY_ACT_GELU_TANH, false);
    else if (vy_act_is_runtime(act)) VY_GO(VY_ACT_RUNTIME, false);
    else VY_FAIL(VY_ERR_ARG, "%s: unknown activation %d", who, act);
  } else {
    if (act == VY_ACT_NONE || !gradpre) VY_GO(VY_ACT_NONE, true);
    else if (act == VY_ACT_GELU_ERF) VY_GO(VY_ACT_GELU_ERF, true);
    else if (act == VY_ACT_GELU_TANH) VY_GO(VY_ACT_GELU_TANH, true);
    else if (vy_act_is_runtime(act) && ep.pre_deriv) VY_GO(VY_ACT_NONE, true);
    else if (vy_act_is_runtime(act)) VY_GO(VY_ACT_RUNTIME, true);
    else VY_FAIL(VY_ERR_ARG, "%s: unknown activation %d", who, act);
  }
#undef VY_GO
  VY_CHECK_LAUNCH(who);
  return VY_OK;
}

template <typename T>
int qkv_impl(const void* x, int64_t ldx, const void* w, int64_t ldw, const void* bias,
             const float* cos_tab, const float* sin_tab, int64_t pos0, void* q, int64_t q_sb,
             int64_t q_sh, int64_t q_sl, void* k, int64_t k_sb, int64_t k_sh, int64_t k_sl, void* v,
             int64_t v_sb, int64_t v_sh, int64_t v_sl, int64_t B, int64_t L, int64_t K, int h, int hk,
             int dh, hipStream_t st, const int* pos_dev = nullptr) {
  const char* who = "vy_qkv_rope_fwd";
  const int64_t M = B * L, N = (int64_t)(h + 2 * hk) * dh;
  if (int rc = check_operands<T>(who, x, ldx, w, ldw, M, N, K)) return rc;
  if (!q || !k || !v) VY_FAIL(VY_ERR_ARG, "%s: null output", who);
  if (h <= 0 || hk <= 0 || h % hk) VY_FAIL(VY_ERR_ARG, "%s: h=%d must be a positive multiple of hk=%d", who, h, hk);
  if (dh % 4) VY_FAIL(VY_ERR_ARG, "%s: head_dim %d must be a multiple of 4", who, dh);
  if ((cos_tab == nullptr) != (sin_tab == nullptr)) VY_FAIL(VY_ERR_ARG, "%s: cos/sin must both be given", who);
  const size_t qa = 4 * sizeof(T);
  const int64_t strides[] = {q_sb, q_sh, q_sl, k_sb, k_sh, k_sl, v_sb, v_sh, v_sl};
  for (int64_t s : strides)
    if (s % 4) VY_FAIL(VY_ERR_ARG, "%s: output strides must be multiples of 4 elements", who);
  if (!aligned_to(q, qa) || !aligned_to(k, qa) || !aligned_to(v, qa) || (bias && !aligned_to(bias, qa)))
    VY_FAIL(VY_ERR_ARG, "%s: outputs/bias must be 4-element aligned", who);
  EpiQkv<T> eq;
  eq.bias = (const T*)bias; eq.cos_tab = cos_tab; eq.sin_tab = sin_tab; eq.pos0 = pos0;
  eq.q = (T*)q; eq.q_sb = q_sb; eq.q_sh = q_sh; eq.q_sl = q_sl;
  eq.k = (T*)k; eq.k_sb = k_sb; eq.k_sh = k_sh; eq.k_sl = k_sl;
  eq.v = (T*)v; eq.v_sb = v_sb; eq.v_sh = v_sh; eq.v_sl = v_sl;
  eq.L = (int)L; eq.nq = h * dh; eq.nkv = hk * dh; eq.dh = dh; eq.pos_dev = pos_dev;
  const bool fuse = cos_tab && sizeof(T) == 2 && dh == 64;
  eq.rope = fuse ? 1 : 0;
  {
    bool v8 = dh % 8 == 0 && aligned_to(q, 16) && aligned_to(k, 16) && aligned_to(v, 16);
    for (int64_t st_ : strides) v8 = v8 && (st_ % 8 == 0);
    eq.vec8 = v8 ? 1 : 0;
  }
  EpiPlain<T> ep{};
  if constexpr (sizeof(T) == 2)
    launch_bf16<1, VY_ACT_NONE, false>((const bf16*)x, ldx, (const bf16*)w, ldw, M, N, K,
                                       *reinterpret_cast<EpiPlain<bf16>*>(&ep), *reinterpret_cast<EpiQkv<bf16>*>(&eq), st);
  else
    launch_f32<1, VY_ACT_NONE, false>((const float*)x, ldx, (const float*)w, ldw, M, N, K,
                                      *reinterpret_cast<EpiPlain<float>*>(&ep), *reinterpret_cast<EpiQkv<float>*>(&eq), st);
  VY_CHECK_LAUNCH(who);
  if (cos_tab && !fuse) {
    if (pos_dev) VY_FAIL(VY_ERR_UNSUPPORTED, "%s: device-side position needs the fused RoPE path (bf16, dh == 64)", who);
    const int vdt = sizeof(T) == 2 ? VY_BF16 : VY_F32;
    if (int rc = vy_rope_qk(q, q_sb, q_sh, q_sl, h, k, k_sb, k_sh, k_sl, hk, cos_tab, sin_tab, pos0, B, L, dh, vdt,
                            (hipStream_t)st)) return rc;
  }
  return VY_OK;
}

}

extern "C" int vy_linear_fwd(const void* x, int64_t ldx, const void* w, int64_t ldw, const void* bias,
                             const void* residual, int64_t ldr, void* y, int64_t ldy, void* pre_out,
                             int64_t M, int64_t N, int64_t K, int act, int dtype, void* stream) {
  hipStream_t st = (hipStream_t)stream;
  if (dtype == VY_BF16)
    return linear_impl<bf16>(x, ldx, w, ldw, bias, residual, ldr, nullptr, 0, y, ldy, pre_out, M, N, K, act, false, st, "vy_linear_fwd");
  if (dtype == VY_F32)
    return linear_impl<float>(x, ldx, w, ldw, bias, residual, ldr, nullptr, 0, y, ldy, pre_out, M, N, K, act, false, st, "vy_linear_fwd");
  VY_FAIL(VY_ERR_ARG, "vy_linear_fwd: bad dtype %d", dtype);
}

extern "C" int vy_linear_dropout_fwd(const void* x, int64_t ldx, const void* w, int64_t ldw, const void* bias,
                                     const void* residual, int64_t ldr, void* y, int64_t ldy, int64_t M, int64_t N,
                                     int64_t K, float p_drop, uint64_t seed, uint64_t offset, int dtype, void* stream) {
  hipStream_t st = (hipStream_t)stream;
  if (!(p_drop >= 0.f && p_drop <= 1.f)) VY_FAIL(VY_ERR_ARG, "vy_linear_dropout_fwd: p=%g outside [0, 1]", (double)p_drop);
  const VyDrop d = vy_make_drop(p_drop, seed, offset);
  if (dtype == VY_BF16)
    return linear_impl<bf16>(x, ldx, w, ldw, bias, residual, ldr, nullptr, 0, y, ldy, nullptr, M, N, K, VY_ACT_NONE, false, st, "vy_linear_dropout_fwd", nullptr, 0, d);
  if (dtype == VY_F32)
    return linear_impl<float>(x, ldx, w, ldw, bias, residual, ldr, nullptr, 0, y, ldy, nullptr, M, N, K, VY_ACT_NONE, false, st, "vy_linear_dropout_fwd", nullptr, 0, d);
  VY_FAIL(VY_ERR_ARG, "vy_linear_dropout_fwd: bad dtype %d", dtype);
}

extern "C" int vy_linear_dgrad(const void* dy, int64_t lddy, const void* wt, int64_t ldwt, const void* pre,
                               int64_t ldpre, int act, const void* add_to, int64_t ldadd, const void* add_to2,
                               int64_t ldadd2, void* dx, int64_t lddx, int64_t M, int64_t N, int64_t K, int dtype,
                               void* stream) {
  hipStream_t st = (hipStream_t)stream;
  if (dtype == VY_BF16)
    return linear_impl<bf16>(dy, lddy, wt, ldwt, nullptr, add_to, ldadd, pre, ldpre, dx, lddx, nullptr, M, K, N, act, true, st, "vy_linear_dgrad", add_to2, ldadd2);
  if (dtype == VY_F32)
    return linear_impl<float>(dy, lddy, wt, ldwt, nullptr, add_to, ldadd, pre, ldpre, dx, lddx, nullptr, M, K, N, act, true, st, "vy_linear_dgrad", add_to2, ldadd2);
  VY_FAIL(VY_ERR_ARG, "vy_linear_dgrad: bad dtype %d", dtype);
}

extern "C" int vy_qkv_rope_fwd(const void* x, int64_t ldx, const void* w, int64_t ldw, const void* bias,
                               const float* cos_tab, const float* sin_tab, int64_t pos0, void* q,
                               int64_t q_sb, int64_t q_sh, int64_t q_sl, void* k, int64_t k_sb,
                               int64_t k_sh, int64_t k_sl, void* v, int64_t v_sb, int64_t v_sh,
                               int64_t v_sl, int64_t B, int64_t L, int64_t K, int h, int hk, int dh,
                               int dtype, void* stream) {
  hipStream_t st = (hipStream_t)stream;
  if (dtype == VY_BF16)
    return qkv_impl<bf16>(x, ldx, w, ldw, bias, cos_tab, sin_tab, pos0, q, q_sb, q_sh, q_sl, k, k_sb, k_sh, k_sl, v, v_sb, v_sh, v_sl, B, L, K, h, hk, dh, st);
  if (dtype == VY_F32)
    return qkv_impl<float>(x, ldx, w, ldw, bias, cos_tab, sin_tab, pos0, q, q_sb, q_sh, q_sl, k, k_sb, k_sh, k_sl, v, v_sb, v_sh, v_sl, B, L, K, h, hk, dh, st);
  VY_FAIL(VY_ERR_ARG, "vy_qkv_rope_fwd: bad dtype %d", dtype);
}

int64_t vy_splitk_ws_floats(int64_t N) { return 8 * 32 * N; }

extern "C" int vy_debug_set_gemm_variant(int v) { g_gemm_variant = v; return 0; }
extern "C" int vy_workspace_set(void* stream, void* ws, int64_t bytes) {
  if (bytes < 0 || (ws && ((uintptr_t)ws & 255))) VY_FAIL(VY_ERR_ARG, "vy_workspace_set: bad workspace (256-byte aligned, bytes >= 0)");
  std::lock_guard<std::mutex> lk(g_ws_mu);
  hipStream_t st = (hipStream_t)stream;
  for (int i = 0; i < g_ws_n; ++i)
    if (g_ws[i].st == st) {
      if (ws && bytes) { g_ws[i].p = ws; g_ws[i].bytes = bytes; }
      else { g_ws[i] = g_ws[g_ws_n - 1]; --g_ws_n; }
      return VY_OK;
    }
  if (!ws || !bytes) return VY_OK;
  if (g_ws_n == 16) {
    for (int i = 1; i < 16; ++i) g_ws[i - 1] = g_ws[i];
    --g_ws_n;
  }
  g_ws[g_ws_n++] = WsEntry{st, ws, bytes};
  return VY_OK;
}
extern "C" int vy_set_concurrent_chains(int n) {
  if (n < 1 || n > 8) VY_FAIL(VY_ERR_ARG, "vy_set_concurrent_chains: n = %d (1..8)", n);
  g_chains = n;
  return VY_OK;
}

extern "C" int vy_debug_gemm_clock(unsigned long long* out3) {
  unsigned long long z[6] = {0, 0, 0, 0, 0, 0};
  if (hipMemcpyFromSymbol(out3, HIP_SYMBOL(vy_gemm_clk), sizeof(z)) != hipSuccess) return 1;
  return hipMemcpyToSymbol(HIP_SYMBOL(vy_gemm_clk), z, sizeof(z)) != hipSuccess;
}
int vy_linear_res_ln_skinny(const void* x, int64_t ldx, const void* w, int64_t ldw, const void* bias,
                            const void* residual, int64_t ldr, const void* gamma, const void* beta, float eps,
                            void* y, int64_t ldy, float* part, int64_t M, int64_t N, int64_t K, void* stream) {
  const char* who = "vy_linear_res_ln_skinny";
  if (!x || !w || !gamma || !beta || !y || !part) VY_FAIL(VY_ERR_ARG, "%s: null operand", who);
  if (M < 1 || M > 32 || N % 32 || K % 16 || N > 8192) VY_FAIL(VY_ERR_UNSUPPORTED, "%s: needs M <= 32, N %% 32 == 0 (<= 8192), K %% 16 == 0", who);
  if (ldx % 8 || ldw % 8 || ldy % 8 || (residual && ldr % 8)) VY_FAIL(VY_ERR_ARG, "%s: strides must be multiples of 8", who);
  hipStream_t st = (hipStream_t)stream;
  const int nsteps = (int)(K / 16), nwg = (int)(N / 32);
  int ksplit = (256 + nwg - 1) / nwg;
  if (ksplit > 8) ksplit = 8;
  if (ksplit > nsteps / 8) ksplit = nsteps / 8;
  if (ksplit < 1) ksplit = 1;
  int spw = (nsteps + ksplit - 1) / ksplit;
  spw = (spw + 3) / 4 * 4;
  ksplit = (nsteps + spw - 1) / spw;
  hipLaunchKernelGGL(gemm_skinny_splitk_kernel, dim3((unsigned)nwg, (unsigned)ksplit), dim3(256), 0, st, (const bf16*)x,
                     ldx, (const bf16*)w, ldw, (int)M, (int)N, (int)K, spw, part);
  VY_CHECK_LAUNCH(who);
  static const int row_fin = [] { const char* e = getenv("VY_DECODE_ROW_FINISH"); return e ? atoi(e) : 1; }();
  if (row_fin && N % 4 == 0) {
    const int qpt = (int)vy_cdiv(N / 4, 256);
#define ROW_GO(Q)                                                                                               \
    hipLaunchKernelGGL((splitk_finish_ln_row_kernel<Q>), dim3((unsigned)M), dim3(256), 0, st, part, ksplit, (int)M, (int)N, \
                       (const bf16*)bias, (const bf16*)residual, ldr, (const bf16*)gamma, (const bf16*)beta, (bf16*)y, ldy, eps)
    if (qpt <= 1) ROW_GO(1);
    else if (qpt <= 2) ROW_GO(2);
    else if (qpt <= 4) ROW_GO(4);
    else ROW_GO(8);
#undef ROW_GO
    VY_CHECK_LAUNCH(who);
    return VY_OK;
  }
  const int nch = (int)(N / 8);
  const dim3 grid((unsigned)((M + 3) / 4)), block(256);
#define FIN_GO(CH)                                                                                               \
  hipLaunchKernelGGL((splitk_finish_ln_kernel<CH>), grid, block, 0, st, part, ksplit, (int)M, (int)N, (const bf16*)bias, \
                     (const bf16*)residual, ldr, (const bf16*)gamma, (const bf16*)beta, (bf16*)y, ldy, eps)
  if (nch <= 64) FIN_GO(1);
  else if (nch <= 128) FIN_GO(2);
  else if (nch <= 256) FIN_GO(4);
  else if (nch <= 512) FIN_GO(8);
  else FIN_GO(16);
#undef FIN_GO
  VY_CHECK_LAUNCH(who);
  return VY_OK;
}

#define VY_NORM_PRESCALED ((const void*)(intptr_t)-1)
static bool gemv_ok(const void* x, int64_t ldx, const void* w, int64_t ldw, int64_t M, int64_t K) {
  return M >= 1 && M <= 4 && K % 8 == 0 && ldx % 8 == 0 && ldw % 8 == 0 && ((uintptr_t)x % 16 == 0) && ((uintptr_t)w % 16 == 0);
}
int vy_gemv_norm(const void* x, int64_t ldx, const void* w, int64_t ldw, const void* bias, const void* norm_w, float eps,
                 const void* residual, int64_t ldr, void* y, int64_t ldy, int64_t M, int64_t N, int64_t K, void* stream) {
// ... 80 lines not shown
```

vyomai_amd/csrc/vy_misc.hip:

```cpp
#include "vy_common.h"
#include <stdarg.h>
#include <string.h>

static thread_local char g_err[512] = "";
void vy_set_error(const char* fmt, ...) {
  va_list ap;
  va_start(ap, fmt);
  vsnprintf(g_err, sizeof(g_err), fmt, ap);
  va_end(ap);
}
extern "C" const char* vy_last_error(void) { return g_err; }
extern "C" int vy_abi_version(void) { return 5; }

namespace {

template <typename T, int CH>
__global__ __launch_bounds__(256) void layernorm_fwd_kernel(const T* __restrict__ x, int64_t ldx,
                                                            const T* __restrict__ gamma,
                                                            const T* __restrict__ beta, T* __restrict__ y,
                                                            int64_t ldy, float* __restrict__ mean_out,
                                                            float* __restrict__ rstd_out, int64_t M, int N,
                                                            float eps) {
  constexpr int VEC = Chunk<T>::VEC;
  const int lane = threadIdx.x & 63;
// ... 704 lines not shown
    if (c < nch) {
      bf16x8 o;
#pragma unroll
      for (int e = 0; e < 8; ++e) {
        const int col = c * 8 + e;
        float g = 0.f;
        if (col < V) g = p.grad(s, __expf((float)v[i][e] - l), col == label ? 1.f : 0.f);
        o[e] = (bf16)g;
      }
      *reinterpret_cast<bf16x8*>(row + (int64_t)c * 8) = o;
    }
  }
}

int row_check(const char* fn, bool ptrs, const void* logits, int64_t ld, int64_t M, int64_t V, int dtype, const char* pair) {
  if (!ptrs || M <= 0 || V <= 0) VY_FAIL(VY_ERR_ARG, "%s: bad arguments", fn);
  if (pair) {
    if (dtype != VY_BF16) VY_FAIL(VY_ERR_UNSUPPORTED, "%s: bf16 only (use %s)", fn, pair);
    if (V > 65536) VY_FAIL(VY_ERR_UNSUPPORTED, "%s: V=%ld exceeds the 65536 columns a workgroup keeps in registers (use %s)", fn, (long)V, pair);
    if (ld % 8 || ld < vy_cdiv(V, 8) * 8 || (uintptr_t)logits % 16) VY_FAIL(VY_ERR_ARG, "%s: rows must be 16-byte aligned and cover the padded width", fn);
    return VY_OK;
  }
  const int vec = dtype == VY_BF16 ? 8 : 4;
  if (ld % vec || ld < vy_cdiv(V, vec) * vec) VY_FAIL(VY_ERR_ARG, "%s: row stride must be a multiple of %d and cover the padded row", fn, vec);
  if (dtype != VY_BF16 && dtype != VY_F32) VY_FAIL(VY_ERR_ARG, "%s: bad dtype %d", fn, dtype);
  return VY_OK;
}

template <typename P>
int row_lse(const char* fn, bool ptrs, const void* logits, int64_t ld, const int64_t* labels, const P& p, float* lse,
            int64_t M, int64_t V, int32_t* err, int dtype, void* stream) {
  if (const int rc = row_check(fn, ptrs && logits && labels && lse, logits, ld, M, V, dtype, nullptr)) return rc;
  const dim3 grid((unsigned)M), block(256);
  if (dtype == VY_BF16) hipLaunchKernelGGL((row_lse_kernel<bf16, P>), grid, block, 0, (hipStream_t)stream, (const bf16*)logits, ld, labels, p, lse, (int)V, err);
  else hipLaunchKernelGGL((row_lse_kernel<float, P>), grid, block, 0, (hipStream_t)stream, (const float*)logits, ld, labels, p, lse, (int)V, err);
  VY_CHECK_LAUNCH(fn);
  return VY_OK;
}

template <typename P>
int row_grad(const char* fn, bool ptrs, void* logits, int64_t ld, const int64_t* labels, const P& p, const float* lse,
             int64_t M, int64_t V, int dtype, void* stream) {
  if (const int rc = row_check(fn, ptrs && logits && labels && lse, logits, ld, M, V, dtype, nullptr)) return rc;
  const dim3 grid((unsigned)M), block(256);
  if (dtype == VY_BF16) hipLaunchKernelGGL((row_grad_kernel<bf16, P>), grid, block, 0, (hipStream_t)stream, (bf16*)logits, ld, labels, p, lse, (int)V);
  else hipLaunchKernelGGL((row_grad_kernel<float, P>), grid, block, 0, (hipStream_t)stream, (float*)logits, ld, labels, p, lse, (int)V);
  VY_CHECK_LAUNCH(fn);
  return VY_OK;
}

template <typename P>
int row_fused(const char* fn, bool ptrs, void* logits, int64_t ld, const int64_t* labels, const P& p, float* lse,
              int64_t M, int64_t V, int32_t* err, int dtype, void* stream) {
  if (const int rc = row_check(fn, ptrs && logits && labels && lse, logits, ld, M, V, dtype, P::kPair)) return rc;
  hipLaunchKernelGGL((row_fused_kernel<P>), dim3((unsigned)M), dim3(1024), 0, (hipStream_t)stream, (bf16*)logits, ld, labels, p, lse, (int)V, err);
  VY_CHECK_LAUNCH(fn);
  return VY_OK;
}

template <typename T>
int ln_fwd_dispatch(const void* x, int64_t ldx, const void* gamma, const void* beta, void* y, int64_t ldy,
                    float* mean, float* rstd, int64_t M, int64_t N, float eps, hipStream_t st) {
  constexpr int VEC = Chunk<T>::VEC;
  if (N % VEC || ldx % VEC || ldy % VEC) VY_FAIL(VY_ERR_ARG, "vy_layernorm_fwd: N/ld must be multiples of %d", VEC);
  const int nch = (int)(N / VEC);
  const dim3 grid((unsigned)vy_cdiv(M, 4)), block(256);
#define LN_GO(CH)                                                                                       \
  hipLaunchKernelGGL((layernorm_fwd_kernel<T, CH>), grid, block, 0, st, (const T*)x, ldx, (const T*)gamma, \
                     (const T*)beta, (T*)y, ldy, mean, rstd, M, (int)N, eps)
  if (nch <= 64) LN_GO(1);
  else if (nch <= 128) LN_GO(2);
  else if (nch <= 256) LN_GO(4);
  else if (nch <= 512) LN_GO(8);
  else if (nch <= 1024) LN_GO(16);
  else VY_FAIL(VY_ERR_UNSUPPORTED, "vy_layernorm_fwd: N=%ld too wide", (long)N);
#undef LN_GO
  VY_CHECK_LAUNCH("vy_layernorm_fwd");
  return VY_OK;
}

template <typename T>
int ln_bwd_dispatch(const void* dy, int64_t lddy, const void* x, int64_t ldx, const void* gamma,
                    const float* mean, const float* rstd, void* dx, int64_t lddx, float* dgamma,
                    float* dbeta, float beta, float* ws, int64_t M, int64_t N, hipStream_t st) {
  constexpr int VEC = Chunk<T>::VEC;
  if (N % VEC || ldx % VEC || lddy % VEC || lddx % VEC) VY_FAIL(VY_ERR_ARG, "vy_layernorm_bwd: N/ld must be multiples of %d", VEC);
  const int nch = (int)(N / VEC);
  const int WB = (int)vy_layernorm_bwd_ws_rows(M);
  const int W = WB * 4;
  const dim3 grid((unsigned)WB), block(256);
#define LN_GO(CH)                                                                                        \
  hipLaunchKernelGGL((layernorm_bwd_kernel<T, CH>), grid, block, 0, st, (const T*)dy, lddy, (const T*)x, ldx, \
                     (const T*)gamma, mean, rstd, (T*)dx, lddx, ws, M, (int)N, W)
  if (nch <= 64) LN_GO(1);
  else if (nch <= 128) LN_GO(2);
  else if (nch <= 256) LN_GO(4);
  else VY_FAIL(VY_ERR_UNSUPPORTED, "vy_layernorm_bwd: N=%ld too wide", (long)N);
#undef LN_GO
  VY_CHECK_LAUNCH("vy_layernorm_bwd");
  if (beta != 0.f && beta != 1.f) VY_FAIL(VY_ERR_ARG, "vy_layernorm_bwd: beta must be 0 or 1");
  const int acc = beta == 1.f;
  const int slices = WB >= 64 ? 16 : 1;
  const int rps = (int)vy_cdiv(WB, slices);
  hipLaunchKernelGGL(colsum_partials_kernel, dim3((unsigned)vy_cdiv(N, 64), (unsigned)slices), dim3(256), 0, st, ws, WB,
                     (int)N, dgamma, dbeta, rps, acc);
  VY_CHECK_LAUNCH("vy_layernorm_bwd(colsum)");
  if (slices > 1) {
    hipLaunchKernelGGL(colsum_finish_kernel, dim3((unsigned)vy_cdiv(N, 256)), dim3(256), 0, st, ws, WB, (int)N, dgamma,
                       dbeta, rps, acc);
    VY_CHECK_LAUNCH("vy_layernorm_bwd(colsum finish)");
  }
  return VY_OK;
}

}

extern "C" int vy_layernorm_fwd(const void* x, int64_t ldx, const void* gamma, const void* beta, void* y,
                                int64_t ldy, float* mean, float* rstd, int64_t M, int64_t N, float eps,
                                int dtype, void* stream) {
  if (!x || !gamma || !beta || !y || M <= 0 || N <= 0) VY_FAIL(VY_ERR_ARG, "vy_layernorm_fwd: bad arguments");
  hipStream_t st = (hipStream_t)stream;
  if (dtype == VY_BF16) return ln_fwd_dispatch<bf16>(x, ldx, gamma, beta, y, ldy, mean, rstd, M, N, eps, st);
  if (dtype == VY_F32) return ln_fwd_dispatch<float>(x, ldx, gamma, beta, y, ldy, mean, rstd, M, N, eps, st);
  VY_FAIL(VY_ERR_ARG, "vy_layernorm_fwd: bad dtype %d", dtype);
}

extern "C" int vy_rmsnorm_fwd(const void* x, int64_t ldx, const void* w, void* y, int64_t ldy, int64_t M, int64_t N,
                              float eps, float w_offset, int dtype, void* stream) {
  if (!x || !w || !y || M <= 0 || N <= 0) VY_FAIL(VY_ERR_ARG, "vy_rmsnorm_fwd: bad arguments");
  hipStream_t st = (hipStream_t)stream;
  const int vec = dtype == VY_BF16 ? 8 : 4;
  if (N % vec || ldx % vec || ldy % vec) VY_FAIL(VY_ERR_ARG, "vy_rmsnorm_fwd: N/ld must be multiples of %d", vec);
  const int nch = (int)(N / vec);
  const dim3 grid((unsigned)vy_cdiv(M, 4)), block(256);
#define RMS_GO(T, CH) hipLaunchKernelGGL((rmsnorm_fwd_kernel<T, CH>), grid, block, 0, st, (const T*)x, ldx, (const T*)w, (T*)y, ldy, M, (int)N, eps, w_offset)
#define RMS_DISPATCH(T)                                  \
  if (nch <= 64) RMS_GO(T, 1);                           \
  else if (nch <= 128) RMS_GO(T, 2);                     \
  else if (nch <= 256) RMS_GO(T, 4);                     \
  else if (nch <= 512) RMS_GO(T, 8);                     \
  else if (nch <= 1024) RMS_GO(T, 16);                   \
  else VY_FAIL(VY_ERR_UNSUPPORTED, "vy_rmsnorm_fwd: N=%ld too wide", (long)N)
  if (dtype == VY_BF16) { RMS_DISPATCH(bf16); }
  else if (dtype == VY_F32) { RMS_DISPATCH(float); }
  else VY_FAIL(VY_ERR_ARG, "vy_rmsnorm_fwd: bad dtype %d", dtype);
#undef RMS_DISPATCH
#undef RMS_GO
  VY_CHECK_LAUNCH("vy_rmsnorm_fwd");
  return VY_OK;
}

extern "C" int vy_gated_act_fwd(const void* gate_up, int64_t ldg, void* out, int64_t ldo, int64_t M, int64_t I, int act,
                                int dtype, void* stream) {
  if (!gate_up || !out || M <= 0 || I <= 0) VY_FAIL(VY_ERR_ARG, "vy_gated_act_fwd: bad arguments");
  if (dtype != VY_BF16 && dtype != VY_F32) VY_FAIL(VY_ERR_ARG, "vy_gated_act_fwd: bad dtype %d", dtype);
  if (act != VY_ACT_GELU_ERF && act != VY_ACT_GELU_TANH && !vy_act_is_runtime(act))
    VY_FAIL(VY_ERR_ARG, "vy_gated_act_fwd: unsupported act %d", act);
  hipStream_t st = (hipStream_t)stream;
  const int vec = dtype == VY_BF16 ? 8 : 4;
  if (I % vec || ldg % vec || ldo % vec) VY_FAIL(VY_ERR_ARG, "vy_gated_act_fwd: I/ld must be multiples of %d", vec);
  const int64_t want = vy_cdiv(M * (I / vec), 256);
  const dim3 grid((unsigned)(want < 8192 ? want : 8192)), block(256);
#define GA_GO(T, A) hipLaunchKernelGGL((gated_act_kernel<T, A>), grid, block, 0, st, (const T*)gate_up, ldg, (T*)out, ldo, M, (int)I, act)
  if (dtype == VY_BF16 && act == VY_ACT_GELU_TANH) GA_GO(bf16, VY_ACT_GELU_TANH);
  else if (dtype == VY_BF16 && act == VY_ACT_GELU_ERF) GA_GO(bf16, VY_ACT_GELU_ERF);
  else if (dtype == VY_F32 && act == VY_ACT_GELU_TANH) GA_GO(float, VY_ACT_GELU_TANH);
  else if (dtype == VY_F32 && act == VY_ACT_GELU_ERF) GA_GO(float, VY_ACT_GELU_ERF);
  else if (dtype == VY_BF16) GA_GO(bf16, VY_ACT_RUNTIME);
  else GA_GO(float, VY_ACT_RUNTIME);
#undef GA_GO
  VY_CHECK_LAUNCH("vy_gated_act_fwd");
  return VY_OK;
}

extern "C" int64_t vy_layernorm_bwd_ws_rows(int64_t M) {
  static const int64_t cap = [] { const char* e = getenv("VY_LNBWD_WB"); return e ? (int64_t)atoi(e) : (int64_t)512; }();
  const int64_t b = (M + 3) / 4;
  return b < 1 ? 1 : (b > cap ? cap : b);
}

extern "C" int vy_layernorm_bwd(const void* dy, int64_t lddy, const void* x, int64_t ldx, const void* gamma,
                                const float* mean, const float* rstd, void* dx, int64_t lddx, float* dgamma,
                                float* dbeta, float beta, float* ws, int64_t M, int64_t N, int dtype,
                                void* stream) {
  if (!dy || !x || !gamma || !mean || !rstd || !dx || !ws || M <= 0 || N <= 0)
    VY_FAIL(VY_ERR_ARG, "vy_layernorm_bwd: bad arguments");
  hipStream_t st = (hipStream_t)stream;
  if (dtype == VY_BF16) return ln_bwd_dispatch<bf16>(dy, lddy, x, ldx, gamma, mean, rstd, dx, lddx, dgamma, dbeta, beta, ws, M, N, st);
  if (dtype == VY_F32) return ln_bwd_dispatch<float>(dy, lddy, x, ldx, gamma, mean, rstd, dx, lddx, dgamma, dbeta, beta, ws, M, N, st);
  VY_FAIL(VY_ERR_ARG, "vy_layernorm_bwd: bad dtype %d", dtype);
}

int vy_rope_qk(void* q, int64_t q_sb, int64_t q_sh, int64_t q_sl, int hq, void* k, int64_t k_sb, int64_t k_sh,
               int64_t k_sl, int hk, const float* cos_tab, const float* sin_tab, int64_t pos0, int64_t B, int64_t L, int dh,
               int dtype, hipStream_t st) {
  if (!q || !k || !cos_tab || !sin_tab || (dh & 1)) VY_FAIL(VY_ERR_ARG, "vy_rope_qk: bad arguments");
  const int64_t total = B * (hq > hk ? hq : hk) * L * (dh / 2);
  const dim3 grid((unsigned)vy_cdiv(total, 256), 2), block(256);
  if (dtype == VY_BF16)
    hipLaunchKernelGGL(rope2_kernel<bf16>, grid, block, 0, st, (bf16*)q, q_sb, q_sh, q_sl, hq, (bf16*)k, k_sb, k_sh, k_sl, hk,
                       cos_tab, sin_tab, pos0, B, L, dh);
  else if (dtype == VY_F32)
    hipLaunchKernelGGL(rope2_kernel<float>, grid, block, 0, st, (float*)q, q_sb, q_sh, q_sl, hq, (float*)k, k_sb, k_sh, k_sl,
                       hk, cos_tab, sin_tab, pos0, B, L, dh);
  else VY_FAIL(VY_ERR_ARG, "vy_rope_qk: bad dtype %d", dtype);
  VY_CHECK_LAUNCH("vy_rope_qk");
  return VY_OK;
}

extern "C" int vy_rope_fwd(void* x, int64_t sb, int64_t sh, int64_t sl, const float* cos_tab,
                           const float* sin_tab, int64_t pos0, int64_t B, int heads, int64_t L, int dh,
                           int inverse, int dtype, void* stream) {
  if (!x || !cos_tab || !sin_tab || dh % 2 || B <= 0 || heads <= 0 || L <= 0)
    VY_FAIL(VY_ERR_ARG, "vy_rope_fwd: bad arguments");
  hipStream_t st = (hipStream_t)stream;
  const int64_t total = B * heads * L * (dh / 2);
  const dim3 grid((unsigned)vy_cdiv(total, 256)), block(256);
  if (dtype == VY_BF16)
    hipLaunchKernelGGL(rope_kernel<bf16>, grid, block, 0, st, (bf16*)x, sb, sh, sl, cos_tab, sin_tab, pos0, B, heads, L, dh, inverse);
  else if (dtype == VY_F32)
    hipLaunchKernelGGL(rope_kernel<float>, grid, block, 0, st, (float*)x, sb, sh, sl, cos_tab, sin_tab, pos0, B, heads, L, dh, inverse);
  else VY_FAIL(VY_ERR_ARG, "vy_rope_fwd: bad dtype %d", dtype);
  VY_CHECK_LAUNCH("vy_rope_fwd");
  return VY_OK;
}

extern "C" int vy_act_bwd(const void* dy, int64_t lddy, const void* pre, int64_t ldpre, void* dx, int64_t lddx,
                          int64_t M, int64_t N, int act, int dtype, void* stream) {
  if (!dy || !pre || !dx || M <= 0 || N <= 0) VY_FAIL(VY_ERR_ARG, "vy_act_bwd: bad arguments");
  hipStream_t st = (hipStream_t)stream;
  const int vec = dtype == VY_BF16 ? 8 : 4;
  if (N % vec || lddy % vec || ldpre % vec || lddx % vec) VY_FAIL(VY_ERR_ARG, "vy_act_bwd: N/ld must be multiples of %d", vec);
  const int64_t want = vy_cdiv(M * (N / vec), 256);
  const dim3 grid((unsigned)(want < 8192 ? want : 8192)), block(256);
#define AB_GO(T, A) hipLaunchKernelGGL((act_bwd_kernel<T, A>), grid, block, 0, st, (const T*)dy, lddy, (const T*)pre, ldpre, (T*)dx, lddx, M, (int)N)
  if (dtype == VY_BF16 && act == VY_ACT_GELU_ERF) AB_GO(bf16, VY_ACT_GELU_ERF);
  else if (dtype == VY_BF16 && act == VY_ACT_GELU_TANH) AB_GO(bf16, VY_ACT_GELU_TANH);
  else if (dtype == VY_F32 && act == VY_ACT_GELU_ERF) AB_GO(float, VY_ACT_GELU_ERF);
  else if (dtype == VY_F32 && act == VY_ACT_GELU_TANH) AB_GO(float, VY_ACT_GELU_TANH);
#define AB_CODE(A)                                          \
  else if (dtype == VY_BF16 && act == A) AB_GO(bf16, A);    \
  else if (dtype == VY_F32 && act == A) AB_GO(float, A);
  AB_CODE(VY_ACT_SILU) AB_CODE(VY_ACT_TANH) AB_CODE(VY_ACT_SIGMOID) AB_CODE(VY_ACT_RELU6) AB_CODE(VY_ACT_LEAKY_RELU)
#undef AB_CODE
  else VY_FAIL(VY_ERR_ARG, "vy_act_bwd: unsupported act %d / dtype %d", act, dtype);
#undef AB_GO
  VY_CHECK_LAUNCH("vy_act_bwd");
  return VY_OK;
}

extern "C" int vy_xent_fwd(const void* logits, int64_t ld, const int64_t* labels, int64_t ignore_index, float* lse,
                           float* loss_sum, float* count, int64_t M, int64_t V, int32_t* err_flag, int dtype,
                           void* stream) {
  return row_lse("vy_xent_fwd", loss_sum && count, logits, ld, labels,
                 XentRow<true>{ignore_index, nullptr, nullptr, loss_sum, count}, lse, M, V, err_flag, dtype, stream);
}

extern "C" int vy_xent_bwd(void* logits, int64_t ld, const int64_t* labels, int64_t ignore_index, const float* lse,
                           const float* gscale, const float* count, int64_t M, int64_t V, int dtype, void* stream) {
  return row_grad("vy_xent_bwd", gscale && count, logits, ld, labels,
                  XentRow<false>{ignore_index, gscale, count, nullptr, nullptr}, lse, M, V, dtype, stream);
}

extern "C" int vy_xent_fused(void* logits, int64_t ld, const int64_t* labels, int64_t ignore_index, float* lse,
                             float* loss_sum, const float* count, const float* gscale, int64_t M, int64_t V,
                             int32_t* err_flag, int dtype, void* stream) {
  return row_fused("vy_xent_fused", loss_sum && count && gscale, logits, ld, labels,
                   XentRow<false>{ignore_index, gscale, count, loss_sum, nullptr}, lse, M, V, err_flag, dtype, stream);
}

extern "C" int vy_xent_sample_fwd(const void* logits, int64_t ld, const int64_t* labels, int64_t ignore_index,
                                  float* lse, float* loss_sum, float* count, int64_t* sampled, float inv_temperature,
                                  uint64_t seed, uint64_t offset, int64_t M, int64_t V, int32_t* err_flag, int dtype,
                                  void* stream) {
  XentSampleRow<true> p{{ignore_index, nullptr, nullptr, loss_sum, count}, sampled, inv_temperature, vy_make_noise(seed, offset)};
// ... 306 lines not shown
```

vyomai_amd/ops.py:

```python
from __future__ import annotations

import math
from typing import Optional, Tuple

import torch

from . import _lib
from ._lib import call, dtype_code

Tensor = torch.Tensor




class _Lanes:
    active = False
    side: Optional[torch.cuda.Stream] = None
    fork_ev: Optional[torch.cuda.Event] = None
    join_ev: Optional[torch.cuda.Event] = None
    B = L = B0 = 0
    dirty = False
    keep: list = []
    streams = {}


class lanes:

    def __init__(self, B: int, L: int, enabled: bool = True):
        self.on = bool(enabled) and B >= 2 and not _Lanes.active and torch.cuda.is_available()
        self.B, self.L = B, L

    def __enter__(self):
        if self.on:
            dev = torch.cuda.current_device()
            st = _Lanes.streams.get(dev)
            if st is None:
                st = _Lanes.streams[dev] = (torch.cuda.Stream(), torch.cuda.Event(), torch.cuda.Event())
            _Lanes.side, _Lanes.fork_ev, _Lanes.join_ev = st
            _Lanes.B, _Lanes.L, _Lanes.B0 = self.B, self.L, self.B // 2
            _Lanes.active, _Lanes.dirty, _Lanes.keep = True, False, []
            call("vy_set_concurrent_chains", 2)
        return self

    def __exit__(self, *exc):
        if self.on:
            _lanes_join()
            _Lanes.active = False
            call("vy_set_concurrent_chains", 1)
            if _Lanes.keep:
                _Lanes.keep = []
        return False


def _lanes_join() -> None:
    if _Lanes.active and _Lanes.dirty:
        _Lanes.join_ev.record(_Lanes.side)
        torch.cuda.current_stream().wait_event(_Lanes.join_ev)
        _Lanes.dirty = False


def _lane_plan(rows: Optional[int] = None, batches: Optional[int] = None, keep=()):
    main = torch.cuda.current_stream()
    if _Lanes.active:
        if rows is not None and rows == _Lanes.B * _Lanes.L:
            cut, n = _Lanes.B0 * _Lanes.L, rows
        elif batches is not None and batches == _Lanes.B:
            cut, n = _Lanes.B0, batches
        else:
            cut = None
        if cut is not None:
            _Lanes.fork_ev.record(main)
            _Lanes.side.wait_event(_Lanes.fork_ev)
            _Lanes.dirty = True
            if keep:
                _Lanes.keep.extend(t for t in keep if t is not None)
            return [(0, cut, main.cuda_stream), (cut, n - cut, _Lanes.side.cuda_stream)]
        _lanes_join()
    n = rows if rows is not None else batches
    return [(0, n, main.cuda_stream)]


def _stream() -> int:
    _lanes_join()
    return torch.cuda.current_stream().cuda_stream


# ... 144 lines not shown
    B, h, _, dh = q.shape
    hk = k.shape[1]
    out = torch.empty((B, 1, h * dh), dtype=q.dtype, device=q.device)
    if scale is None:
        scale = 1.0 / math.sqrt(dh)
    call("vy_attn_decode", q.data_ptr(), q.stride(0), q.stride(1),
         k.data_ptr(), k.stride(0), k.stride(1), k.stride(2),
         v.data_ptr(), v.stride(0), v.stride(1), v.stride(2),
         out.data_ptr(), out.stride(0), B, h, hk, S, dh, float(scale), dtype_code(q.dtype), _stream())
    return out


def layernorm(x: Tensor, gamma: Tensor, beta: Tensor, eps: float,
              save_stats: bool = False) -> Tuple[Tensor, Optional[Tensor], Optional[Tensor]]:
    _need_gpu(x, gamma, beta)
    x2 = _rows(x)
    M, N = x2.shape
    y = torch.empty((M, N), dtype=x.dtype, device=x.device)
    mean = rstd = None
    if save_stats:
        mean = torch.empty(M, dtype=torch.float32, device=x.device)
        rstd = torch.empty(M, dtype=torch.float32, device=x.device)
    whole = _Lanes.active and x2.data_ptr() != x.data_ptr()
    for m0, m, st in ([(0, M, _stream())] if whole else _lane_plan(rows=M, keep=(x2, y, mean, rstd, gamma, beta))):
        call("vy_layernorm_fwd", _at(x2, m0), x2.stride(0), gamma.data_ptr(), beta.data_ptr(),
             _at(y, m0), y.stride(0), _at(mean, m0), _at(rstd, m0), m, N, float(eps), dtype_code(x.dtype), st)
    return y.view(x.shape), mean, rstd


def rope_(x: Tensor, cos: Tensor, sin: Tensor, pos0: int = 0, inverse: bool = False) -> Tensor:
    _need_gpu(x, cos, sin)
    B, heads, L, dh = x.shape
    assert x.stride(3) == 1
    call("vy_rope_fwd", x.data_ptr(), x.stride(0), x.stride(1), x.stride(2), cos.data_ptr(),
         sin.data_ptr(), pos0, B, heads, L, dh, 1 if inverse else 0, dtype_code(x.dtype), _stream())
    return x


def rope_tables(head_dim: int, max_pos: int, device) -> Tuple[Tensor, Tensor]:
    inv_freq = 1.0 / (10000 ** (torch.arange(0, head_dim, 2).float() / head_dim))
    t = torch.arange(max_pos).type_as(inv_freq)
    ang = torch.einsum("i,j->ij", t, inv_freq)
    return ang.cos().contiguous().to(device), ang.sin().contiguous().to(device)




def linear_dgrad(dy: Tensor, wt: Tensor, pre: Optional[Tensor] = None, act: int = _lib.ACT_NONE,
                 add_to: Optional[Tensor] = None, out: Optional[Tensor] = None,
                 add_to2: Optional[Tensor] = None) -> Tensor:
    _need_gpu(dy, wt, pre, add_to, add_to2)
    if add_to is None and add_to2 is not None:
        add_to, add_to2 = add_to2, None
    d2 = _rows(dy)
    M, N = d2.shape
    K = wt.shape[0]
    assert wt.shape[1] == N and wt.stride(1) == 1
    if out is None:
        out = torch.empty((*dy.shape[:-1], K), dtype=dy.dtype, device=dy.device)
    o2 = _rows(out)
    p2 = _rows(pre) if pre is not None else None
    a2 = _rows(add_to) if add_to is not None else None
    b2 = _rows(add_to2) if add_to2 is not None else None
    _mid_ws(M)
    call("vy_linear_dgrad", d2.data_ptr(), d2.stride(0), wt.data_ptr(), wt.stride(0), _ptr(p2),
         p2.stride(0) if p2 is not None else 0, act, _ptr(a2), a2.stride(0) if a2 is not None else 0,
         _ptr(b2), b2.stride(0) if b2 is not None else 0,
         o2.data_ptr(), o2.stride(0), M, N, K, dtype_code(dy.dtype), _stream())
    return out


def linear_wgrad(dy: Tensor, x: Tensor, dw: Tensor, db: Optional[Tensor], accumulate: bool,
                 alpha: Optional[Tensor] = None) -> None:
    _need_gpu(dy, x, dw, db, alpha)
    assert alpha is None or (alpha.dtype == torch.float32 and alpha.numel() == 1)
    d2, x2 = _rows(dy), _rows(x)
    M, N = d2.shape
    K = x2.shape[1]
    assert dw.dtype == torch.float32 and dw.shape == (N, K) and dw.stride(1) == 1
    call("vy_linear_wgrad", d2.data_ptr(), d2.stride(0), x2.data_ptr(), x2.stride(0), dw.data_ptr(),
         dw.stride(0), _ptr(db), 1.0 if accumulate else 0.0, _ptr(alpha), M, N, K, dtype_code(dy.dtype), _stream())


def linear_wgrad_grouped(items) -> None:
    import ctypes as C
    n = len(items)
    assert 1 <= n <= 8
    arr = (_lib.VyWgradDesc * n)()
    dt = None
    for i, (dy, x, dw, db) in enumerate(items):
        _need_gpu(dy, x, dw, db)
        d2, x2 = _rows(dy), _rows(x)
        M, N = d2.shape
        K = x2.shape[1]
        assert x2.shape[0] == M and dw.dtype == torch.float32 and dw.shape == (N, K) and dw.stride(1) == 1
        assert db is None or (db.dtype == torch.float32 and db.numel() == N)
        assert dt is None or dt == dy.dtype
        dt = dy.dtype
        a = arr[i]
        a.dy, a.lddy, a.x, a.ldx = d2.data_ptr(), d2.stride(0), x2.data_ptr(), x2.stride(0)
        a.dw, a.lddw, a.db = dw.data_ptr(), dw.stride(0), _ptr(db)
        a.M, a.N, a.K = M, N, K
    call("vy_linear_wgrad_grouped", C.cast(arr, C.c_void_p), n, dtype_code(dt), _stream())


def layernorm_bwd(dy: Tensor, x: Tensor, gamma: Tensor, mean: Tensor, rstd: Tensor, dgamma: Tensor,
                  dbeta: Tensor, accumulate: bool) -> Tensor:
    _need_gpu(dy, x, gamma, mean, rstd, dgamma, dbeta)
    d2, x2 = _rows(dy), _rows(x)
    M, N = x2.shape
    dx = torch.empty((M, N), dtype=x.dtype, device=x.device)
    W = _lib.load().vy_layernorm_bwd_ws_rows(M)
    ws = torch.empty((2 * W * N,), dtype=torch.float32, device=x.device)
    call("vy_layernorm_bwd", d2.data_ptr(), d2.stride(0), x2.data_ptr(), x2.stride(0), gamma.data_ptr(),
         mean.data_ptr(), rstd.data_ptr(), dx.data_ptr(), dx.stride(0), dgamma.data_ptr(), dbeta.data_ptr(),
         1.0 if accumulate else 0.0, ws.data_ptr(), M, N, dtype_code(x.dtype), _stream())
    return dx.view(x.shape)


def attention_bwd(q, k, v, out, dout, lse, dq, dk, dv, *, causal: bool, start_pos: int = 0,
                  keypad: Optional[Tensor] = None, scale: Optional[float] = None,
                  cos: Optional[Tensor] = None, sin: Optional[Tensor] = None, rope_pos0: int = 0,
                  delta: Optional[Tensor] = None) -> None:
    _need_gpu(q, k, v, out, dout, lse, dq, dk, dv, keypad)
    B, h, L, dh = q.shape
    hk, S = k.shape[1], k.shape[2]
    kind = (_lib.MASK_CAUSAL if causal else 0) | (_lib.MASK_KEYPAD if keypad is not None else 0)
    if scale is None:
        scale = 1.0 / math.sqrt(dh)
    assert out.stride() == dout.stride() and out.stride(2) == 1
    if delta is None:
        delta = torch.empty((B, h, L), dtype=torch.float32, device=q.device)
    assert delta.dtype == torch.float32 and delta.is_contiguous() and delta.shape == (B, h, L)
    call("vy_attn_bwd", q.data_ptr(), q.stride(0), q.stride(1), q.stride(2),
         k.data_ptr(), k.stride(0), k.stride(1), k.stride(2),
         v.data_ptr(), v.stride(0), v.stride(1), v.stride(2),
         out.data_ptr(), dout.data_ptr(), out.stride(0), out.stride(1), lse.data_ptr(), delta.data_ptr(),
         dq.data_ptr(), dq.stride(0), dq.stride(1), dq.stride(2),
         dk.data_ptr(), dk.stride(0), dk.stride(1), dk.stride(2),
         dv.data_ptr(), dv.stride(0), dv.stride(1), dv.stride(2),
         kind, start_pos, _ptr(keypad), keypad.stride(0) if keypad is not None else 0,
         _ptr(cos), _ptr(sin), rope_pos0,
         B, h, hk, L, S, dh, float(scale), dtype_code(q.dtype), _stream())


def adamw_step(p: Tensor, g: Tensor, m: Tensor, v: Tensor, p_bf16: Optional[Tensor], lr: float,
               beta1: float, beta2: float, eps: float, weight_decay: float, step: int,
               grad_scale: float = 1.0, scale_dev: Optional[Tensor] = None, gate: Optional[Tensor] = None) -> None:
    _need_gpu(p, g, m, v, p_bf16, scale_dev, gate)
    assert scale_dev is None or (scale_dev.dtype == torch.float32 and scale_dev.numel() == 1)
    if gate is None:
        call("vy_adamw_step", p.data_ptr(), g.data_ptr(), m.data_ptr(), v.data_ptr(), _ptr(p_bf16), p.numel(),
             lr, beta1, beta2, eps, weight_decay, step, grad_scale, _ptr(scale_dev), _stream())
    else:
        assert gate.dtype == torch.float32 and gate.numel() == 1
        call("vy_adamw_step_gated", p.data_ptr(), g.data_ptr(), m.data_ptr(), v.data_ptr(), _ptr(p_bf16), p.numel(),
             lr, beta1, beta2, eps, weight_decay, step, grad_scale, _ptr(scale_dev), gate.data_ptr(), _stream())


def sumsq(x: Tensor) -> Tensor:
    _need_gpu(x)
    assert x.dtype == torch.float32 and x.is_contiguous()
    out = torch.empty(1, dtype=torch.float32, device=x.device)
    ws = torch.empty(1024, dtype=torch.float32, device=x.device)
    call("vy_sumsq", x.data_ptr(), x.numel(), out.data_ptr(), ws.data_ptr(), _stream())
    return out[0]


def dropout(x: Tensor, p: float, seed: int, offset: int, out: Optional[Tensor] = None) -> Tensor:
    _need_gpu(x, out)
    x2 = _rows(x)
    if out is None:
        out = torch.empty_like(x2)
        ret = out.view(x.shape)
    else:
        ret = out
    o2 = _rows(out)
    call("vy_dropout", x2.data_ptr(), x2.stride(0), o2.data_ptr(), o2.stride(0), x2.shape[0], x2.shape[1],
         float(p), int(seed), int(offset), dtype_code(x.dtype), _stream())
    return ret


def transpose(x: Tensor, out: Optional[Tensor] = None) -> Tensor:
    _need_gpu(x)
    R, C = x.shape
    if out is None:
# ... 371 lines not shown
```

Before: 862,600 tokens/s.

## Fold LayerNorm gamma/beta column sums into grouped wgrad launch; prefetch epilogue residuals

LayerNorm backward now runs only the row pass and writes partial sums to a workspace. The gamma/beta column reduction is deferred into the grouped weight-gradient kernel as extra trailing blocks, which removes two small kernel launches per LayerNorm and lets the reductions overlap with GEMM tiles. Separately, the GEMM epilogue now prefetches residual and gradient-pre-activation tiles before the shared-memory sync and skips bounds checks on full tiles. The costs are larger workspace lifetimes, more register pressure in the epilogue, and more complex deferral bookkeeping.

```diff
diff --git a/include/vyom_hip.h b/include/vyom_hip.h
--- a/include/vyom_hip.h
+++ b/include/vyom_hip.h
@@ -117,11 +117,22 @@
 } vy_wgrad_desc;
 int vy_linear_wgrad_grouped(const vy_wgrad_desc* descs, int32_t n, int dtype, void* stream);
 
+typedef struct vy_colsum_desc {
+  float* ws; int32_t W, N;
+  float* out0; float* out1;
+  int32_t acc;
+} vy_colsum_desc;
+int vy_linear_wgrad_grouped_cs(const vy_wgrad_desc* descs, int32_t n, const vy_colsum_desc* cs, int32_t ncs, int dtype,
+                               void* stream);
+
 int64_t vy_layernorm_bwd_ws_rows(int64_t M);
 int vy_layernorm_bwd(const void* dy, int64_t lddy, const void* x, int64_t ldx, const void* gamma,
                      const float* mean, const float* rstd, void* dx, int64_t lddx, float* dgamma,
                      float* dbeta, float beta, float* ws, int64_t M, int64_t N, int dtype,
                      void* stream);
+int vy_layernorm_bwd_partial(const void* dy, int64_t lddy, const void* x, int64_t ldx, const void* gamma,
+                             const float* mean, const float* rstd, void* dx, int64_t lddx, float* ws, int64_t M,
+                             int64_t N, int dtype, void* stream);
 
 int vy_attn_bwd(const void* q, int64_t q_sb, int64_t q_sh, int64_t q_sl,
                 const void* k, int64_t k_sb, int64_t k_sh, int64_t k_sl,
diff --git a/vyomai_amd/_lib.py b/vyomai_amd/_lib.py
--- a/vyomai_amd/_lib.py
+++ b/vyomai_amd/_lib.py
@@ -38,6 +38,8 @@
     "vy_linear_dgrad": [_p, _i64, _p, _i64, _p, _i64, _i, _p, _i64, _p, _i64, _p, _i64, _i64, _i64, _i64, _i, _p],
     "vy_linear_wgrad": [_p, _i64, _p, _i64, _p, _i64, _p, _f, _p, _i64, _i64, _i64, _i, _p],
     "vy_linear_wgrad_grouped": [_p, _i, _i, _p],
+    "vy_linear_wgrad_grouped_cs": [_p, _i, _p, _i, _i, _p],
+    "vy_layernorm_bwd_partial": [_p, _i64, _p, _i64, _p, _p, _p, _p, _i64, _p, _i64, _i64, _i, _p],
     "vy_layernorm_bwd": [_p, _i64, _p, _i64, _p, _p, _p, _p, _i64, _p, _p, _f, _p, _i64, _i64, _i, _p],
     "vy_attn_bwd": [_p, _i64, _i64, _i64, _p, _i64, _i64, _i64, _p, _i64, _i64, _i64,
                     _p, _p, _i64, _i64, _p, _p,
@@ -85,6 +87,10 @@
 class VyWgradDesc(C.Structure):
     _fields_ = [("dy", _p), ("lddy", _i64), ("x", _p), ("ldx", _i64), ("dw", _p), ("lddw", _i64), ("db", _p),
                 ("M", _i64), ("N", _i64), ("K", _i64)]
+
+
+class VyColsumDesc(C.Structure):
+    _fields_ = [("ws", _p), ("W", C.c_int32), ("N", C.c_int32), ("out0", _p), ("out1", _p), ("acc", C.c_int32)]
 
 
 class VyomHipError(RuntimeError):
diff --git a/vyomai_amd/autograd_train.py b/vyomai_amd/autograd_train.py
--- a/vyomai_amd/autograd_train.py
+++ b/vyomai_amd/autograd_train.py
@@ -108,7 +108,7 @@
     TILES = int(os.environ.get("VY_WGRAD_GROUP_TILES", "100"))
 
     def __init__(self):
-        self.items, self.tiles, self.armed = [], 0, False
+        self.items, self.colsums, self.tiles, self.armed = [], [], 0, False
 
     def wants(self, dy, w, alpha) -> bool:
         if alpha is not None or not _GROUP_WGRADS:
@@ -124,18 +124,30 @@
         for p in members:
             p._vy_deferred = True
         self.tiles += -(-dw.shape[0] // 256) * -(-dw.shape[1] // 256)
+        self._arm()
+        if self.tiles >= self.TILES or len(self.items) == 8:
+            self.flush()
+
+    def add_colsum(self, ws, dgamma, dbeta, members) -> None:
+        self.colsums.append((ws, dgamma, dbeta, members))
+        for p in members:
+            p._vy_deferred = True
+        self._arm()
+        if len(self.colsums) == 8:
+            self.flush()
+
+    def _arm(self) -> None:
         if not self.armed:
             torch.autograd.Variable._execution_engine.queue_callback(self._end_of_backward)
             self.armed = True
-        if self.tiles >= self.TILES or len(self.items) == 8:
-            self.flush()
 
     def flush(self) -> None:
-        items, self.items, self.tiles = self.items, [], 0
-        if not items:
+        items, colsums, self.items, self.colsums, self.tiles = self.items, self.colsums, [], [], 0
+        if not items and not colsums:
             return
-        ops.linear_wgrad_grouped([(dy, x, dw, db) for dy, x, dw, db, _ in items])
-        for *_, members in items:
+        ops.linear_wgrad_grouped([(dy, x, dw, db) for dy, x, dw, db, _ in items] +
+                                 [ops.ColSum(ws, dg, db, True, torch.bfloat16) for ws, dg, db, _ in colsums])
+        for *_, members in items + colsums:
             for p in members:
                 p._vy_deferred = False
             _notify(*members)
@@ -145,16 +157,17 @@
         self.flush()
 
     def discard(self) -> None:
-        for *_, members in self.items:
+        for *_, members in self.items + self.colsums:
             for p in members:
                 p._vy_deferred = False
-        self.items, self.tiles, self.armed = [], 0, False
+        self.items, self.colsums, self.tiles, self.armed = [], [], 0, False
 
 
 _GROUP_WGRADS = os.environ.get("VY_WGRAD_GROUP", "1") != "0"
 _DEFER_RESIDUALS = os.environ.get("VY_DEFER_RESIDUALS", "1") != "0"
 _GROUP_MIN_ROWS = int(os.environ.get("VY_WGRAD_GROUP_ROWS", "2048"))
 _GROUP_QKV = os.environ.get("VY_WGRAD_GROUP_QKV", "1") != "0"
+_GROUP_LN_COLSUMS = os.environ.get("VY_LN_COLSUM_GROUP", "1") != "0"
 _wgrad_group = _WgradGroup()
 
 
@@ -175,6 +188,11 @@
 def _ln_bwd(dy, x, ln_w, ln_b, mean, rstd):
     dt = x.dtype
     if _direct(ln_w) and _direct(ln_b):
+        if (_GROUP_LN_COLSUMS and _GROUP_WGRADS and dt == torch.bfloat16
+                and x.numel() // x.shape[-1] >= _GROUP_MIN_ROWS):
+            dx, ws = ops.layernorm_bwd_partial(dy, x, _shadow(ln_w, dt), mean, rstd)
+            _wgrad_group.add_colsum(ws, ln_w.grad, ln_b.grad, [ln_w, ln_b])
+            return dx, None, None
         dx = ops.layernorm_bwd(dy, x, _shadow(ln_w, dt), mean, rstd, ln_w.grad, ln_b.grad, accumulate=True)
         _notify(ln_w, ln_b)
         return dx, None, None
diff --git a/vyomai_amd/csrc/vy_bwd.hip b/vyomai_amd/csrc/vy_bwd.hip
--- a/vyomai_amd/csrc/vy_bwd.hip
+++ b/vyomai_amd/csrc/vy_bwd.hip
@@ -1,6 +1,7 @@
 #include "vy_attn_tile.h"
 #include <float.h>
 #include <stdlib.h>
+#include <string.h>
 
 namespace {
 
@@ -337,9 +338,72 @@
 };
 struct WgradGroup { WgradItem g[8]; int n; };
 
+struct ColsumItem { const float* ws; float* out0; float* out1; int W, N, rps, acc, blk0; };
+struct ColsumGroup { ColsumItem c[8]; int n; int items; };
+
+__device__ __forceinline__ void colsum_slab_block(const ColsumItem& it, int blk) {
+  __shared__ float red[2][2][4][64];
+  const int tid = threadIdx.x;
+  const int c = tid & 63, g = (tid >> 6) & 3, h = tid >> 8;
+  const int n = blk * 64 + c;
+  const int W = it.W, N = it.N, rps = it.rps;
+  const float* __restrict__ ws = it.ws;
+  const bool one = rps >= W;
+  float ta = 0.f, tb = 0.f;
+  for (int s0 = 0; s0 * rps < W; s0 += 2) {
+    const int w0 = (s0 + h) * rps, w1 = min(W, w0 + rps);
+    float a = 0.f, b = 0.f;
+    if (n < N) {
+      for (int wb = w0 + g; wb < w1; wb += 32) {
+        float av[8], bv[8];
+#pragma unroll
+        for (int i = 0; i < 8; ++i) {
+          const int w = wb + 4 * i;
+          const int wc = w < w1 ? w : wb;
+          av[i] = ws[(int64_t)wc * N + n];
+          bv[i] = ws[(int64_t)(W + wc) * N + n];
+        }
+#pragma unroll
+        for (int i = 0; i < 8; ++i)
+          if (wb + 4 * i < w1) { a += av[i]; b += bv[i]; }
+      }
+    }
+    red[h][0][g][c] = a; red[h][1][g][c] = b;
+    __syncthreads();
+    if (tid < 64) {
+#pragma unroll
+      for (int hh = 0; hh < 2; ++hh)
+        if ((s0 + hh) * rps < W) {
+          const float sa = red[hh][0][0][c] + red[hh][0][1][c] + red[hh][0][2][c] + red[hh][0][3][c];
+          const float sb = red[hh][1][0][c] + red[hh][1][1][c] + red[hh][1][2][c] + red[hh][1][3][c];
+          ta = one ? sa : ta + sa;
+          tb = one ? sb : tb + sb;
+        }
+    }
+    __syncthreads();
+  }
+  if (tid < 64 && n < N) {
+    if (it.out0) it.out0[n] = (it.acc ? it.out0[n] : 0.f) + ta;
+    if (it.out1) it.out1[n] = (it.acc ? it.out1[n] : 0.f) + tb;
+  }
+}
+
 template <int BN, int BKW, int MS, int NS, bool MF16>
-__global__ __launch_bounds__(BN * 2, 1) void wgrad_tn_bf16_grouped_kernel(WgradGroup grp, int diag) {
-  const int id = xcd_remap(blockIdx.x, gridDim.x);
+__global__ __launch_bounds__(BN * 2, 1) void wgrad_tn_bf16_grouped_kernel(WgradGroup grp, ColsumGroup cs, int diag) {
+  if ((int)blockIdx.x >= cs.items) {
+    const int blk = (int)blockIdx.x - cs.items;
+    int d = 0;
+#pragma unroll
+    for (int i = 1; i < 8; ++i)
+      if (i < cs.n && blk >= cs.c[i].blk0) d = i;
+    ColsumItem it = cs.c[0];
+#pragma unroll
+    for (int i = 1; i < 8; ++i)
+      if (d == i) it = cs.c[i];
+    colsum_slab_block(it, blk - it.blk0);
+    return;
+  }
+  const int id = xcd_remap(blockIdx.x, cs.items);
   int d = 0;
 #pragma unroll
   for (int i = 1; i < 8; ++i)
@@ -798,11 +862,17 @@
   return VY_OK;
 }
 
-extern "C" int vy_linear_wgrad_grouped(const vy_wgrad_desc* descs, int32_t n, int dtype, void* stream) {
-  const char* who = "vy_linear_wgrad_grouped";
+static int wgrad_grouped(const char* who, const vy_wgrad_desc* descs, int32_t n, const vy_colsum_desc* cs, int32_t ncs,
+                        int dtype, void* stream) {
   if (dtype != VY_BF16 && dtype != VY_F32) VY_FAIL(VY_ERR_ARG, "%s: bad dtype %d", who, dtype);
-  if (!descs || n <= 0 || n > 8) VY_FAIL(VY_ERR_ARG, "%s: 1..8 descriptors", who);
+  if (n < 0 || n > 8 || (n > 0 && !descs) || ncs < 0 || ncs > 8 || (ncs > 0 && !cs) || n + ncs == 0)
+    VY_FAIL(VY_ERR_ARG, "%s: 1..8 descriptors", who);
+  for (int i = 0; i < ncs; ++i)
+    if (!cs[i].ws || cs[i].W <= 0 || cs[i].N <= 0 || (cs[i].acc != 0 && cs[i].acc != 1))
+      VY_FAIL(VY_ERR_ARG, "%s: column-sum descriptor %d: bad arguments", who, i);
   if (dtype == VY_F32) {
+    for (int i = 0; i < ncs; ++i)
+      if (int rc = vy_ln_colsum(cs[i].ws, cs[i].W, cs[i].N, cs[i].out0, cs[i].out1, cs[i].acc, (hipStream_t)stream)) return rc;
     for (int i = 0; i < n; ++i) {
       const vy_wgrad_desc& d = descs[i];
       if (!d.dy || !d.x || !d.dw || d.M <= 0 || d.N <= 0 || d.K <= 0) VY_FAIL(VY_ERR_ARG, "%s: descriptor %d: bad arguments", who, i);
@@ -820,6 +890,7 @@
   }
   static const int tgt = wgrad_env("VY_WGRAD_GROUP_TARGET", 256);
   WgradGroup grp;
+  memset(&grp, 0, sizeof(grp));
   grp.n = n;
   int64_t items = 0;
   for (int i = 0; i < n; ++i) {
@@ -834,10 +905,32 @@
     items += tiles * sp.splits;
   }
   for (int i = n; i < 8; ++i) grp.g[i] = grp.g[0];
+  ColsumGroup cg;
+  memset(&cg, 0, sizeof(cg));
+  cg.n = ncs; cg.items = (int)items;
+  int64_t blocks = 0;
+  for (int i = 0; i < ncs; ++i) {
+    ColsumItem& c = cg.c[i];
+    c.ws = cs[i].ws; c.out0 = cs[i].out0; c.out1 = cs[i].out1;
+    c.W = cs[i].W; c.N = cs[i].N; c.acc = cs[i].acc;
+    c.rps = (int)vy_cdiv(c.W, vy_ln_colsum_slices(c.W));
+    c.blk0 = (int)blocks;
+    blocks += vy_cdiv(c.N, 64);
+  }
   auto kernel = wgrad_m16() ? wgrad_tn_bf16_grouped_kernel<256, 256, 32, 4, true> : wgrad_tn_bf16_grouped_kernel<256, 256, 32, 4, false>;
-  hipLaunchKernelGGL(kernel, dim3((unsigned)items), dim3(512), 0, (hipStream_t)stream, grp, wgrad_diag());
+  hipLaunchKernelGGL(kernel, dim3((unsigned)(items + blocks)), dim3(512), 0, (hipStream_t)stream, grp, cg, wgrad_diag());
   VY_CHECK_LAUNCH(who);
   return VY_OK;
+}
+
+extern "C" int vy_linear_wgrad_grouped(const vy_wgrad_desc* descs, int32_t n, int dtype, void* stream) {
+  if (!descs || n <= 0 || n > 8) VY_FAIL(VY_ERR_ARG, "vy_linear_wgrad_grouped: 1..8 descriptors");
+  return wgrad_grouped("vy_linear_wgrad_grouped", descs, n, nullptr, 0, dtype, stream);
+}
+
+extern "C" int vy_linear_wgrad_grouped_cs(const vy_wgrad_desc* descs, int32_t n, const vy_colsum_desc* cs, int32_t ncs,
+                                          int dtype, void* stream) {
+  return wgrad_grouped("vy_linear_wgrad_grouped_cs", descs, n, cs, ncs, dtype, stream);
 }
 
 namespace {
diff --git a/vyomai_amd/csrc/vy_common.h b/vyomai_amd/csrc/vy_common.h
--- a/vyomai_amd/csrc/vy_common.h
+++ b/vyomai_amd/csrc/vy_common.h
@@ -83,6 +83,9 @@
 
 static inline int64_t vy_cdiv(int64_t a, int64_t b) { return (a + b - 1) / b; }
 
+static inline int vy_ln_colsum_slices(int WB) { return WB >= 64 ? 16 : 1; }
+int vy_ln_colsum(float* ws, int WB, int N, float* dgamma, float* dbeta, int acc, hipStream_t st);
+
 static __device__ __attribute__((aligned(16))) uint32_t vy_zero16[4] = {0, 0, 0, 0};
 
 __device__ __forceinline__ float vy_gelu_erf(float x) {
diff --git a/vyomai_amd/csrc/vy_gemm.hip b/vyomai_amd/csrc/vy_gemm.hip
--- a/vyomai_amd/csrc/vy_gemm.hip
+++ b/vyomai_amd/csrc/vy_gemm.hip
@@ -53,6 +53,7 @@
   int wt_store;
   int pre_deriv;
   int act;
+  int pf2;
 };
 
 template <typename T, int ACT, bool GRAD>
@@ -261,9 +262,14 @@
 
 int g_chains = 1;
 int g_gemm_variant = -2;
+int g_epi_prefetch = -2;
 inline bool vy_m16_on() {
   static const int v = [] { const char* e = getenv("VY_GEMM_M16"); return e ? atoi(e) : 1; }();
   return v != 0;
+}
+inline int vy_epi_prefetch() {
+  if (g_epi_prefetch == -2) { const char* e = getenv("VY_EPI_PREFETCH"); g_epi_prefetch = e ? (atoi(e) != 0) : 1; }
+  return g_epi_prefetch;
 }
 inline int vy_gemm_variant() {
   if (g_gemm_variant == -2) { const char* e = getenv("VY_GEMM_VARIANT"); g_gemm_variant = e ? atoi(e) : -1; }
@@ -384,11 +390,12 @@
     const bf16* pf_ptr = GRAD ? (ep.gradpre ? ep.gradpre : ep.residual) : ep.residual;
     const int64_t pf_ld = GRAD ? (ep.gradpre ? ep.ldg : ep.ldr) : ep.ldr;
     const bool pf_is_gradpre = GRAD && ep.gradpre != nullptr;
-    auto do_chunk = [&](bf16* __restrict__ dst, bool dual, int pass, int c, bool pf, const bf16x8& p8) {
+    auto do_chunk = [&](bf16* __restrict__ dst, bool dual, int pass, int c, bool pf, const bf16x8& p8, bool pf2,
+                        const bf16x8& rb, const bf16x8& rc, bool fast) __attribute__((always_inline)) {
         const int row = c / CPR, cc = c - row * CPR;
         const int64_t m = m0 + pass * RP + row;
         const int n = n0 + cc * 8;
-        if (m >= M || n >= N) return;
+        if (!fast && (m >= M || n >= N)) return;
         const bf16x8 sv = *reinterpret_cast<const bf16x8*>(et + row * EROW + cc * 16);
         float v[8];
 #pragma unroll
@@ -412,7 +419,7 @@
             for (int e = 0; e < 8; ++e) v[e] = vy_drop_keep(ep.drop, lots, e) ? v[e] * ep.drop.scale : 0.f;
           }
         }
-        if (ep.vec_ok && n + 8 <= N) {
+        if (fast || (ep.vec_ok && n + 8 <= N)) {
           if constexpr (GRAD) {
             if (ep.gradpre) {
               const bf16x8 g = pf ? p8 : *reinterpret_cast<const bf16x8*>(ep.gradpre + m * ep.ldg + n);
@@ -421,12 +428,13 @@
             }
           }
           if (ep.residual) {
-            const bf16x8 r = (pf && !pf_is_gradpre) ? p8 : *reinterpret_cast<const bf16x8*>(ep.residual + m * ep.ldr + n);
+            const bf16x8 r = (pf && !pf_is_gradpre) ? p8
+                             : (pf2 && GRAD) ? rb : *reinterpret_cast<const bf16x8*>(ep.residual + m * ep.ldr + n);
 #pragma unroll
             for (int e = 0; e < 8; ++e) v[e] += (float)r[e];
           }
           if (ep.residual2) {
-            const bf16x8 r = *reinterpret_cast<const bf16x8*>(ep.residual2 + m * ep.ldr2 + n);
+            const bf16x8 r = pf2 ? rc : *reinterpret_cast<const bf16x8*>(ep.residual2 + m * ep.ldr2 + n);
 #pragma unroll
             for (int e = 0; e < 8; ++e) v[e] += (float)r[e];
           }
@@ -451,35 +459,72 @@
         }
     };
     constexpr bool PFK = PF_OK && PASSES == 1 && BM * BN == 256 * 192 && (RP * CPR) % NT == 0;
-    constexpr int ITERS = PFK ? (RP * CPR) / NT : 1;
+    constexpr bool PF2K = (RP * CPR) % NT == 0 && (ACT == VY_ACT_NONE || ACT == VY_ACT_GELU_ERF);
+    constexpr int ITERS = (PFK || PF2K) ? (RP * CPR) / NT : 1;
     bf16x8 pre8[ITERS];
-    const bool pf_on = PFK && pf_ptr != nullptr && ep.vec_ok && m0 + BM <= M && n0 + BN <= N;
+    bf16x8 rb8[GRAD ? ITERS : 1];
+    bf16x8 rc8[ITERS];
+    const bool whole = ep.vec_ok && m0 + BM <= M && n0 + BN <= N;
+    const bool pf_on = PFK && pf_ptr != nullptr && whole;
+    const bool pf2_on = PF2K && ep.pf2 && pf_ptr != nullptr && whole;
+    auto pf_addr = [&](const bf16* p, int64_t ld, int pass, int it) {
+      const int c = tid + it * NT;
+      const int row = c / CPR, cc = c - row * CPR;
+      return reinterpret_cast<const bf16x8*>(p + (int64_t)(m0 + pass * RP + row) * ld + n0 + cc * 8);
+    };
     if constexpr (PFK) {
       if (pf_on) {
 #pragma unroll
-        for (int it = 0; it < ITERS; ++it) {
-          const int c = tid + it * NT;
-          const int row = c / CPR, cc = c - row * CPR;
-          pre8[it] = *reinterpret_cast<const bf16x8*>(pf_ptr + (int64_t)(m0 + row) * pf_ld + n0 + cc * 8);
+        for (int it = 0; it < ITERS; ++it) pre8[it] = *pf_addr(pf_ptr, pf_ld, 0, it);
+      }
+    }
+    auto prefetch_rest = [&](int pass) {
+      if constexpr (PF2K) {
+        if (pf2_on) {
+          if (!pf_on) {
+#pragma unroll
+            for (int it = 0; it < ITERS; ++it) pre8[it] = *pf_addr(pf_ptr, pf_ld, pass, it);
+          }
+          if constexpr (GRAD) {
+            if (pf_is_gradpre && ep.residual) {
+#pragma unroll
+              for (int it = 0; it < ITERS; ++it) rb8[it] = *pf_addr(ep.residual, ep.ldr, pass, it);
+            }
+          }
+          if (ep.residual2) {
+#pragma unroll
+            for (int it = 0; it < ITERS; ++it) rc8[it] = *pf_addr(ep.residual2, ep.ldr2, pass, it);
+          }
         }
       }
-    }
+    };
     auto flush_plain = [&](bf16* __restrict__ dst, bool final_pass, bool dual, int pass) {
       (void)final_pass;
+      if constexpr (PF2K) {
+        if (pf2_on) {
+#pragma unroll
+          for (int it = 0; it < ITERS; ++it)
+            do_chunk(dst, dual, pass, tid + it * NT, true, pre8[it], true, rb8[GRAD ? it : 0], rc8[it], true);
+          return;
+        }
+      }
+      const bf16x8 none{};
       if constexpr (PFK) {
         if (pf_on) {
 #pragma unroll
-          for (int it = 0; it < ITERS; ++it) do_chunk(dst, dual, pass, tid + it * NT, true, pre8[it]);
+          for (int it = 0; it < ITERS; ++it) do_chunk(dst, dual, pass, tid + it * NT, true, pre8[it], false, none, none, false);
           return;
         }
       }
-      const bf16x8 none{};
-      for (int c = tid; c < RP * CPR; c += NT) do_chunk(dst, dual, pass, c, false, none);
+      for (int c = tid; c < RP * CPR; c += NT) do_chunk(dst, dual, pass, c, false, none, false, none, none, false);
     };
     const bool dual = !GRAD && ep.pre != nullptr;
 #pragma unroll 1
     for (int pass = 0; pass < PASSES; ++pass) {
       stage_all(pass);
+      asm volatile("" ::: "memory");
+      __builtin_amdgcn_sched_barrier(0);
+      prefetch_rest(pass);
       __syncthreads();
       flush_plain(ep.y, true, dual, pass);
       if (pass + 1 < PASSES) __syncthreads();
@@ -1737,6 +1782,7 @@
   if (residual2 && !residual) VY_FAIL(VY_ERR_ARG, "%s: add_to2 without add_to", who);
   ep.gradpre = (const T*)gradpre; ep.ldg = ldg; ep.y = (T*)y; ep.ldy = ldy; ep.pre = (T*)pre_out;
   ep.drop = drop;
+  ep.pf2 = vy_epi_prefetch();
   static const int wt_env = [] { const char* e = getenv("VY_GEMM_WT_STORE"); return e ? atoi(e) : 1; }();
   ep.wt_store = (wt_env && (int64_t)M * N * (int64_t)sizeof(T) >= (16 << 20)) ? 1 : 0;
   const int ve = 16 / (int)sizeof(T);
@@ -1878,6 +1924,7 @@
 int64_t vy_splitk_ws_floats(int64_t N) { return 8 * 32 * N; }
 
 extern "C" int vy_debug_set_gemm_variant(int v) { g_gemm_variant = v; return 0; }
+extern "C" int vy_debug_set_epilogue_prefetch(int on) { g_epi_prefetch = on ? 1 : 0; return 0; }
 extern "C" int vy_workspace_set(void* stream, void* ws, int64_t bytes) {
   if (bytes < 0 || (ws && ((uintptr_t)ws & 255))) VY_FAIL(VY_ERR_ARG, "vy_workspace_set: bad workspace (256-byte aligned, bytes >= 0)");
   std::lock_guard<std::mutex> lk(g_ws_mu);
diff --git a/vyomai_amd/csrc/vy_misc.hip b/vyomai_amd/csrc/vy_misc.hip
--- a/vyomai_amd/csrc/vy_misc.hip
+++ b/vyomai_amd/csrc/vy_misc.hip
@@ -810,7 +810,7 @@
 template <typename T>
 int ln_bwd_dispatch(const void* dy, int64_t lddy, const void* x, int64_t ldx, const void* gamma,
                     const float* mean, const float* rstd, void* dx, int64_t lddx, float* dgamma,
-                    float* dbeta, float beta, float* ws, int64_t M, int64_t N, hipStream_t st) {
+                    float* dbeta, float beta, float* ws, int64_t M, int64_t N, hipStream_t st, bool partial = false) {
   constexpr int VEC = Chunk<T>::VEC;
   if (N % VEC || ldx % VEC || lddy % VEC || lddx % VEC) VY_FAIL(VY_ERR_ARG, "vy_layernorm_bwd: N/ld must be multiples of %d", VEC);
   const int nch = (int)(N / VEC);
@@ -826,21 +826,25 @@
   else VY_FAIL(VY_ERR_UNSUPPORTED, "vy_layernorm_bwd: N=%ld too wide", (long)N);
 #undef LN_GO
   VY_CHECK_LAUNCH("vy_layernorm_bwd");
+  if (partial) return VY_OK;
   if (beta != 0.f && beta != 1.f) VY_FAIL(VY_ERR_ARG, "vy_layernorm_bwd: beta must be 0 or 1");
-  const int acc = beta == 1.f;
-  const int slices = WB >= 64 ? 16 : 1;
+  return vy_ln_colsum(ws, WB, (int)N, dgamma, dbeta, beta == 1.f, st);
+}
+
+}
+
+int vy_ln_colsum(float* ws, int WB, int N, float* dgamma, float* dbeta, int acc, hipStream_t st) {
+  const int slices = vy_ln_colsum_slices(WB);
   const int rps = (int)vy_cdiv(WB, slices);
   hipLaunchKernelGGL(colsum_partials_kernel, dim3((unsigned)vy_cdiv(N, 64), (unsigned)slices), dim3(256), 0, st, ws, WB,
-                     (int)N, dgamma, dbeta, rps, acc);
+                     N, dgamma, dbeta, rps, acc);
   VY_CHECK_LAUNCH("vy_layernorm_bwd(colsum)");
   if (slices > 1) {
-    hipLaunchKernelGGL(colsum_finish_kernel, dim3((unsigned)vy_cdiv(N, 256)), dim3(256), 0, st, ws, WB, (int)N, dgamma,
+    hipLaunchKernelGGL(colsum_finish_kernel, dim3((unsigned)vy_cdiv(N, 256)), dim3(256), 0, st, ws, WB, N, dgamma,
                        dbeta, rps, acc);
     VY_CHECK_LAUNCH("vy_layernorm_bwd(colsum finish)");
   }
   return VY_OK;
-}
-
 }
 
 extern "C" int vy_layernorm_fwd(const void* x, int64_t ldx, const void* gamma, const void* beta, void* y,
@@ -919,6 +923,17 @@
   VY_FAIL(VY_ERR_ARG, "vy_layernorm_bwd: bad dtype %d", dtype);
 }
 
+extern "C" int vy_layernorm_bwd_partial(const void* dy, int64_t lddy, const void* x, int64_t ldx, const void* gamma,
+                                        const float* mean, const float* rstd, void* dx, int64_t lddx, float* ws,
+                                        int64_t M, int64_t N, int dtype, void* stream) {
+  if (!dy || !x || !gamma || !mean || !rstd || !dx || !ws || M <= 0 || N <= 0)
+    VY_FAIL(VY_ERR_ARG, "vy_layernorm_bwd_partial: bad arguments");
+  hipStream_t st = (hipStream_t)stream;
+  if (dtype == VY_BF16) return ln_bwd_dispatch<bf16>(dy, lddy, x, ldx, gamma, mean, rstd, dx, lddx, nullptr, nullptr, 0.f, ws, M, N, st, true);
+  if (dtype == VY_F32) return ln_bwd_dispatch<float>(dy, lddy, x, ldx, gamma, mean, rstd, dx, lddx, nullptr, nullptr, 0.f, ws, M, N, st, true);
+  VY_FAIL(VY_ERR_ARG, "vy_layernorm_bwd_partial: bad dtype %d", dtype);
+}
+
 int vy_rope_qk(void* q, int64_t q_sb, int64_t q_sh, int64_t q_sl, int hq, void* k, int64_t k_sb, int64_t k_sh,
                int64_t k_sl, int hk, const float* cos_tab, const float* sin_tab, int64_t pos0, int64_t B, int64_t L, int dh,
                int dtype, hipStream_t st) {
diff --git a/vyomai_amd/ops.py b/vyomai_amd/ops.py
--- a/vyomai_amd/ops.py
+++ b/vyomai_amd/ops.py
@@ -1,7 +1,7 @@
 from __future__ import annotations
 
 import math
-from typing import Optional, Tuple
+from typing import NamedTuple, Optional, Tuple
 
 import torch
 
@@ -312,11 +312,21 @@
          dw.stride(0), _ptr(db), 1.0 if accumulate else 0.0, _ptr(alpha), M, N, K, dtype_code(dy.dtype), _stream())
 
 
+class ColSum(NamedTuple):
+    ws: Tensor
+    dgamma: Tensor
+    dbeta: Tensor
+    accumulate: bool
+    dtype: torch.dtype
+
+
 def linear_wgrad_grouped(items) -> None:
     import ctypes as C
-    n = len(items)
-    assert 1 <= n <= 8
-    arr = (_lib.VyWgradDesc * n)()
+    colsums = [it for it in items if isinstance(it, ColSum)]
+    items = [it for it in items if not isinstance(it, ColSum)]
+    n, ncs = len(items), len(colsums)
+    assert n <= 8 and ncs <= 8 and n + ncs >= 1
+    arr = (_lib.VyWgradDesc * max(n, 1))()
     dt = None
     for i, (dy, x, dw, db) in enumerate(items):
         _need_gpu(dy, x, dw, db)
@@ -331,7 +341,34 @@
         a.dy, a.lddy, a.x, a.ldx = d2.data_ptr(), d2.stride(0), x2.data_ptr(), x2.stride(0)
         a.dw, a.lddw, a.db = dw.data_ptr(), dw.stride(0), _ptr(db)
         a.M, a.N, a.K = M, N, K
-    call("vy_linear_wgrad_grouped", C.cast(arr, C.c_void_p), n, dtype_code(dt), _stream())
+    if not ncs:
+        call("vy_linear_wgrad_grouped", C.cast(arr, C.c_void_p), n, dtype_code(dt), _stream())
+        return
+    cs = (_lib.VyColsumDesc * ncs)()
+    for i, (ws, dgamma, dbeta, accumulate, cdt) in enumerate(colsums):
+        _need_gpu(ws, dgamma, dbeta)
+        dt = cdt if dt is None else dt
+        N = dgamma.numel()
+        assert ws.dtype == torch.float32 and ws.is_contiguous() and ws.numel() % (2 * N) == 0
+        assert dgamma.dtype == torch.float32 and dbeta.dtype == torch.float32 and dbeta.numel() == N
+        assert dgamma.is_contiguous() and dbeta.is_contiguous()
+        c = cs[i]
+        c.ws, c.W, c.N = ws.data_ptr(), ws.numel() // (2 * N), N
+        c.out0, c.out1, c.acc = dgamma.data_ptr(), dbeta.data_ptr(), 1 if accumulate else 0
+    call("vy_linear_wgrad_grouped_cs", C.cast(arr, C.c_void_p) if n else None, n, C.cast(cs, C.c_void_p), ncs,
+         dtype_code(dt), _stream())
+
+
+def layernorm_bwd_partial(dy: Tensor, x: Tensor, gamma: Tensor, mean: Tensor, rstd: Tensor):
+    _need_gpu(dy, x, gamma, mean, rstd)
+    d2, x2 = _rows(dy), _rows(x)
+    M, N = x2.shape
+    dx = torch.empty((M, N), dtype=x.dtype, device=x.device)
+    W = _lib.load().vy_layernorm_bwd_ws_rows(M)
+    ws = torch.empty((2 * W * N,), dtype=torch.float32, device=x.device)
+    call("vy_layernorm_bwd_partial", d2.data_ptr(), d2.stride(0), x2.data_ptr(), x2.stride(0), gamma.data_ptr(),
+         mean.data_ptr(), rstd.data_ptr(), dx.data_ptr(), dx.stride(0), ws.data_ptr(), M, N, dtype_code(x.dtype), _stream())
+    return dx.view(x.shape), ws
 
 
 def layernorm_bwd(dy: Tensor, x: Tensor, gamma: Tensor, mean: Tensor, rstd: Tensor, dgamma: Tensor,
```

After: 885,900 tokens/s, median of 6. 1.03x the previous value.
